# SaeedRahmani/MPC_for_AV_at_Intersection

Hardware: AMD Instinct MI355X
Metric: MPC timesteps/sec (whole node), N=20 horizon, 8-agent intersection, batch=4096 (higher is better)
Workload: dtype f64

## Files before the change

include/mpcx.h:

```cpp
#ifndef MPCX_H
#define MPCX_H
#include <stdint.h>

#ifdef __cplusplus
extern "C" {
#endif

#define MPCX_T_MAX 32
#define MPCX_MAX_PRIM 16
#define MPCX_MAX_OBS 16
#define MPCX_PRED_STEPS_MAX 64
#define MPCX_MAX_REMAINING 1024
#define MPCX_MAX_PATH_LEN 4096
#define MPCX_EGO_FRAMES_MAX 128

enum {
    MPCX_OK = 0,
    MPCX_E_INVALID = -1,
    MPCX_E_LAUNCH = -2,
    MPCX_E_NODEVICE = -3
};

enum { MPCX_QP_OPTIMAL = 0, MPCX_QP_MAXITER = 1, MPCX_QP_INFEASIBLE = 2, MPCX_QP_NUMERIC = 3 };

// ... 27 lines not shown
                            const double *u_warm ,
                            double *x_out , double *u_out ,
                            int32_t *status , int32_t *iters , double *kkt );

int32_t mpcx_mpc_prepare_batch(mpcx_ctx *ctx, int32_t B, const double *state ,
                               const double *u_warm ,
                               const double *path_xyyaw , const double *path_v ,
                               const int32_t *path_off ,
                               const int32_t *path_len , double dl, int32_t *target_ind ,
                               double *xref , uint8_t *reaches_end , double *xbar );
int32_t mpcx_mpc_prepare_batch_ov(mpcx_ctx *ctx, int32_t B, const double *state, const double *u_warm,
                                  const double *path_xyyaw, const double *path_v, const int32_t *path_off, const int32_t *path_len,
                                  double dl, int32_t *target_ind, const double *ov , int64_t ov_stride,
                                  double *xref, uint8_t *reaches_end, double *xbar);
#define MPCX_NO_STOP 999
int32_t mpcx_mpc_prepare_batch_stop(mpcx_ctx *ctx, int32_t B, const double *state, const double *u_warm,
                                    const double *path_xyyaw, const double *path_v, const int32_t *path_off, const int32_t *path_len,
                                    double dl, int32_t *target_ind, const double *ov , int64_t ov_stride,
                                    const int32_t *stop_idx , double v_ref, int32_t *len_seen ,
                                    double *xref, uint8_t *reaches_end, double *xbar);
int32_t mpcx_set_linearisation_passes(mpcx_ctx *ctx, int32_t passes);

typedef struct mpcx_search_model mpcx_search_model;
mpcx_search_model *mpcx_search_model_create(mpcx_ctx *ctx, int32_t n_prim,
                                            const int32_t *tmpl_off , const double *tmpl_xy ,
                                            const double *last_pose , const double *edge_cost ,
                                            int32_t n_obst, const int32_t *hp_off , const double *hp );
void mpcx_search_model_destroy(mpcx_search_model *m);
int32_t mpcx_expand_batch(mpcx_ctx *ctx, const mpcx_search_model *m, int32_t n_nodes, const double *nodes ,
                          const double *nodes_cs ,
                          double *nbr , double *cost , uint8_t *collide );

enum { MPCX_ASTAR_BASE = 0, MPCX_ASTAR_MODIFIED = 1, MPCX_ASTAR_MULTI_LANE = 2, MPCX_ASTAR_ROUNDABOUT = 3, MPCX_ASTAR_SINGLE_LANE = 4 };
enum { MPCX_ASTAR_FOUND = 0, MPCX_ASTAR_EXHAUSTED = 1 , MPCX_ASTAR_CAPACITY = 2, MPCX_ASTAR_MISS = 3,
       MPCX_ASTAR_PATH_CAPACITY = 4 };
typedef struct {
    double start[3];
    double goal_box[4];
    double goal_point[3];
    double allowed_dtheta;
    double wh[5];
    double wc[4];
    const double *hp_norm;
    int32_t variant;
    int32_t max_expansions;
    int32_t ov_off, ov_cnt;
} mpcx_astar_search;
typedef struct {
    int32_t heap_cap, table_cap, log_cap, push_cap, path_cap;
    double *heap, *table, *log, *push_log, *path, *cost, *miss;
    int32_t *status, *n_exp, *n_push, *path_len, *path_prim;
} mpcx_astar_buffers;
int32_t mpcx_astar_batch(mpcx_ctx *ctx, int32_t n_search, const mpcx_search_model *const *models, const mpcx_astar_search *searches,
                         int32_t n_cs, const double *cs_theta, const double *cs_val,
                         int32_t n_ov, const double *ov_key , const double *ov_val , const mpcx_astar_buffers *buffers);

int32_t mpcx_expand_multi_batch(mpcx_ctx *ctx, int32_t n_seg, const mpcx_search_model *const *models, const int32_t *seg_off,
                                const double *nodes , const double *nodes_cs ,
                                double *nbr , double *cost , uint8_t *collide );

typedef struct {
    int32_t pred_steps;
    int32_t frame_window;
    int32_t cutoff_margin;
    int32_t max_path_len;
    double dt, L, radius;
    double circle_centers[4];
    double max_accel, max_speed;
    const double *path_cum;
    double path_cum_err;
    const int32_t *path_first_within;
    const int32_t *plan_cnt;
    const double *plan_disc, *plan_box, *path_disc;
    int32_t plan_cap, plan_steps;
    double plan_dl, plan_radius;
} mpcx_interaction_params;
int32_t mpcx_interaction_batch(mpcx_ctx *ctx, const mpcx_interaction_params *ip, int32_t P,
                               const double *state ,
                               const double *path_xyyaw , const double *path_cs ,
                               const int32_t *path_off , const int32_t *path_len ,
                               const int32_t *prev_cut_len ,
                               int32_t n_obs_pool, const double *obs6 , const int32_t *obs_off ,
                               const int32_t *obs_cnt , const int32_t *obs_skip ,
                               int32_t *traj_idx , int32_t *hit_idx , double *hit_xy ,
                               int32_t *cut_len );

int32_t mpcx_moving_collision_batch(mpcx_ctx *ctx, const mpcx_interaction_params *ip, int32_t P,
                                    const double *ego_xyyaw , const double *ego_cs ,
                                    const int32_t *ego_off , const int32_t *ego_len ,
                                    const double *path_xyyaw , const double *path_cs ,
                                    const int32_t *path_off , const int32_t *path_len ,
                                    int32_t n_obs_pool, const double *obs_xyyaw , const double *obs_cs ,
                                    const int32_t *obs_off , const int32_t *obs_cnt ,
                                    int32_t *hit_idx , double *hit_xy );

int32_t mpcx_transform_batch(mpcx_ctx *ctx, int32_t n_items, int32_t max_pts, const double *nodes ,
                             const int32_t *pts_off , const int32_t *pts_cnt , const double *pts ,
                             double *out );

int32_t mpcx_cutoff_index_batch(mpcx_ctx *ctx, int32_t P, const double *pts , const int32_t *off ,
                                const int32_t *len , const double *xy , double radius, int32_t *out );

int32_t mpcx_predict_obstacles_batch(mpcx_ctx *ctx, int32_t n, int32_t steps, double dt, double L,
                                     const double *obs6 , double *out_xyyaw );

int32_t mpcx_selftest_wave_ops(mpcx_ctx *ctx, const double *in64, double *out322);
int32_t mpcx_selftest_mfma(mpcx_ctx *ctx, const double *A64, const double *B64, double *D256);

int32_t mpcx_plant_step_batch(mpcx_ctx *ctx, int32_t B, double *state , double *u ,
                              const int32_t *status , double *applied );

enum { MPCX_TRAFFIC_TINTERSECTION = 0, MPCX_TRAFFIC_ROUNDABOUT = 1, MPCX_TRAFFIC_ARTERIAL = 2, MPCX_TRAFFIC_TAPE = 3 };
typedef struct {
    int32_t kind;
    int32_t direction;
    int32_t turning;
    int32_t tape_rows, tape_off, tape_stride;
    double speed;
    double offset;
    double counter_dt;
    double model_dt;
    double L;
    double x_turn;
    double arc;
} mpcx_traffic_actor;
int32_t mpcx_traffic_step_batch(mpcx_ctx *ctx, int32_t n_actors, const mpcx_traffic_actor *actors, double *actor_state ,
                                const double *tape , int64_t tape_rows,
                                const int32_t *pool_row , int32_t n_obs_pool, double *obs6 );

typedef struct {
    int32_t P;
    int32_t exchange;
    double dl;
    double *state , *applied , *obs6 ;
    const double *path_xyyaw, *path_cs, *path_v ;
    const int32_t *path_off , *path_len , *obs_off , *obs_cnt , *obs_skip ;
    int32_t *traj_idx , *target_ind , *hit_idx , *cut_len ;
    double *hit_xy , *xref , *xbar ;
    uint8_t *reaches_end ;
    double *x_sol , *u_sol ;
    int32_t *status , *iters ;
    double *kkt ;
    int32_t n_inst, agents_local;
    double *obs_local ;
    int32_t n_actors, pool_rows ;
    const mpcx_traffic_actor *actors ;
    double *actor_state ;
    const double *tape ;
    const int32_t *actor_row , *ego_row ;
    int64_t tape_rows;
} mpcx_closed_loop;
int32_t mpcx_closed_loop_run(mpcx_ctx *ctx, const mpcx_interaction_params *ip, const mpcx_closed_loop *cl,
                             int32_t n_steps, int32_t use_graph);
int32_t mpcx_closed_loop_stats(mpcx_ctx *ctx, int64_t *out4 , int32_t reset);
int32_t mpcx_closed_loop_queue(mpcx_ctx *ctx, int32_t P, int32_t *order , int32_t *keyslot );
int32_t mpcx_interaction_prediction(mpcx_ctx *ctx, int32_t rows, int32_t steps, double *out );

typedef struct {
    int32_t capacity;
    int32_t reserved;
    double goal_dis, stop_speed;
    double *rows_f64 ;
    int32_t *rows_i32 ;
    int32_t *steps , *goal_step , *contact_step , *flags ;
    double *min_clearance ;
} mpcx_run_log;
int32_t mpcx_record_step_batch(mpcx_ctx *ctx, const mpcx_interaction_params *ip, int32_t P,
                               const double *state , const double *applied , const double *x_sol ,
                               const double *path_xyyaw , const int32_t *path_off , const int32_t *path_len ,
                               const int32_t *target_ind , const int32_t *cut_len , const int32_t *traj_idx ,
                               const int32_t *hit_idx , const int32_t *status , const int32_t *iters ,
                               int32_t n_obs_pool, const double *obs6 , const int32_t *obs_off ,
                               const int32_t *obs_cnt , const int32_t *obs_skip , const mpcx_run_log *log);
int32_t mpcx_record_step_batch_goal(mpcx_ctx *ctx, const mpcx_interaction_params *ip, int32_t P,
                                    const double *state, const double *applied, const double *x_sol,
                                    const double *path_xyyaw, const int32_t *path_off, const int32_t *path_len,
                                    const int32_t *target_ind, const int32_t *cut_len, const int32_t *traj_idx,
                                    const int32_t *hit_idx, const int32_t *status, const int32_t *iters,
                                    int32_t n_obs_pool, const double *obs6, const int32_t *obs_off,
                                    const int32_t *obs_cnt, const int32_t *obs_skip, const int32_t *goal_len ,
                                    const mpcx_run_log *log);
int32_t mpcx_closed_loop_run_logged(mpcx_ctx *ctx, const mpcx_interaction_params *ip, const mpcx_closed_loop *cl,
                                    const mpcx_run_log *log, int32_t n_steps, int32_t use_graph);
enum { MPCX_STOP_CUT = 0, MPCX_STOP_SPEED = 1 };
typedef struct {
    int32_t stop_mode;
    int32_t reserved;
    double v_ref;
    int32_t *prev_len;
} mpcx_closed_loop_opts;
int32_t mpcx_closed_loop_run_opts(mpcx_ctx *ctx, const mpcx_interaction_params *ip, const mpcx_closed_loop *cl,
                                  const mpcx_run_log *log , const mpcx_closed_loop_opts *opts ,
                                  int32_t n_steps, int32_t use_graph);

typedef struct {
    int32_t *done;
    int32_t *steps_driven;
    double goal_dis, stop_speed;
} mpcx_retire;
int32_t mpcx_closed_loop_run_retire(mpcx_ctx *ctx, const mpcx_interaction_params *ip, const mpcx_closed_loop *cl,
                                    const mpcx_run_log *log , const mpcx_closed_loop_opts *opts ,
                                    const mpcx_retire *retire , int32_t n_steps, int32_t use_graph);

typedef struct {
    int32_t *absent;
    int32_t n_rows;
    int32_t reserved;
} mpcx_scene;
int32_t mpcx_closed_loop_run_scene(mpcx_ctx *ctx, const mpcx_interaction_params *ip, const mpcx_closed_loop *cl,
                                   const mpcx_run_log *log , const mpcx_closed_loop_opts *opts ,
                                   const mpcx_retire *retire , const mpcx_scene *scene ,
                                   int32_t n_steps, int32_t use_graph);

typedef struct {
    int32_t *wait;
    int32_t *entered_step;
    int32_t *clock;
    int32_t reserved;
    double gap;
} mpcx_admit;
int32_t mpcx_closed_loop_run_admit(mpcx_ctx *ctx, const mpcx_interaction_params *ip, const mpcx_closed_loop *cl,
                                   const mpcx_run_log *log , const mpcx_closed_loop_opts *opts ,
                                   const mpcx_retire *retire , const mpcx_scene *scene ,
                                   const mpcx_admit *admit , int32_t n_steps, int32_t use_graph);
int32_t mpcx_admit_step_batch(mpcx_ctx *ctx, const mpcx_interaction_params *ip, int32_t P, const double *state ,
                              const int32_t *obs_off , const int32_t *obs_cnt , const int32_t *obs_skip ,
                              int32_t *done , int32_t n_obs_pool, int32_t *absent ,
                              int32_t n_actors, const mpcx_traffic_actor *actors , const double *actor_state ,
                              const double *tape , int64_t tape_rows, const int32_t *actor_row ,
                              const mpcx_admit *admit);

typedef struct {
    int32_t generations;
    int32_t reserved;
    const double  *start_state;
    const int32_t *start_idx;
    const int32_t *due;
    int32_t *served;
    int32_t *ep_i32;
    double  *ep_f64;
} mpcx_respawn;
int32_t mpcx_closed_loop_run_respawn(mpcx_ctx *ctx, const mpcx_interaction_params *ip, const mpcx_closed_loop *cl,
                                     const mpcx_run_log *log , const mpcx_closed_loop_opts *opts ,
                                     const mpcx_retire *retire , const mpcx_scene *scene ,
                                     const mpcx_admit *admit , const mpcx_respawn *respawn ,
                                     int32_t n_steps, int32_t use_graph);
int32_t mpcx_respawn_step_batch(mpcx_ctx *ctx, int32_t P, double *state , double *applied , double *u_sol ,
                                int32_t *traj_idx , int32_t *target_ind , int32_t *cut_len , int32_t *iters ,
                                int32_t *prev_len , const int32_t *obs_skip , int32_t n_obs_pool,
                                const mpcx_run_log *log , const mpcx_retire *retire, const mpcx_admit *admit,
                                const mpcx_respawn *respawn);

typedef struct {
    int32_t n_routes;
    int32_t reserved;
    const int32_t *route_off;
    const int32_t *route_len;
    const int32_t *route_of;
    const double  *start_state;
    const int32_t *start_idx;
    int32_t *path_off;
    int32_t *path_len;
} mpcx_routes;
int32_t mpcx_closed_loop_run_routes(mpcx_ctx *ctx, const mpcx_interaction_params *ip, const mpcx_closed_loop *cl,
                                    const mpcx_run_log *log , const mpcx_closed_loop_opts *opts ,
                                    const mpcx_retire *retire , const mpcx_scene *scene ,
                                    const mpcx_admit *admit , const mpcx_respawn *respawn ,
                                    const mpcx_routes *routes , int32_t n_steps, int32_t use_graph);
int32_t mpcx_respawn_step_batch_routes(mpcx_ctx *ctx, int32_t P, double *state , double *applied , double *u_sol ,
                                       int32_t *traj_idx , int32_t *target_ind , int32_t *cut_len , int32_t *iters ,
                                       int32_t *prev_len , const int32_t *obs_skip , int32_t n_obs_pool,
                                       const mpcx_run_log *log , const mpcx_retire *retire, const mpcx_admit *admit,
                                       const mpcx_respawn *respawn, const mpcx_routes *routes , int32_t max_path_len);
int32_t mpcx_episode_summary(mpcx_ctx *ctx, int32_t P, int32_t A, int32_t G, int32_t R, const int32_t *served ,
                             const int32_t *ep_i32 , const double *ep_f64 , int64_t *out_i64 ,
                             double *out_f64 );

enum { MPCX_PRECEDENCE_FIXED = 1, MPCX_PRECEDENCE_ENTRY = 2 };
typedef struct {
    int32_t *prec;
    double *stand;
    int32_t n_rows;
    int32_t mode;
} mpcx_precedence;
int32_t mpcx_closed_loop_run_precedence(mpcx_ctx *ctx, const mpcx_interaction_params *ip, const mpcx_closed_loop *cl,
                                        const mpcx_run_log *log , const mpcx_closed_loop_opts *opts ,
                                        const mpcx_retire *retire , const mpcx_scene *scene ,
                                        const mpcx_admit *admit , const mpcx_respawn *respawn ,
                                        const mpcx_routes *routes , const mpcx_precedence *precedence ,
                                        int32_t n_steps, int32_t use_graph);
int32_t mpcx_admit_step_batch_precedence(mpcx_ctx *ctx, const mpcx_interaction_params *ip, int32_t P, const double *state ,
                                         const int32_t *obs_off , const int32_t *obs_cnt , const int32_t *obs_skip ,
                                         int32_t *done , int32_t n_obs_pool, int32_t *absent ,
                                         int32_t n_actors, const mpcx_traffic_actor *actors , const double *actor_state ,
                                         const double *tape , int64_t tape_rows, const int32_t *actor_row ,
                                         const mpcx_admit *admit, const mpcx_precedence *precedence );

#define MPCX_SIGNAL_GROUPS_MAX 16
typedef struct {
    const int32_t *path_stop;
    const int32_t *path_group;
    const int32_t *plan_cycle;
    const int32_t *plan_amber;
    const int32_t *plan_green;
    const int32_t *plan_of;
    int32_t *tick;
// ... 70 lines not shown
```

mpc_for_av_at_intersection_amd/_lib.py:

```python
import ctypes as C
import os

_HERE = os.path.dirname(os.path.abspath(__file__))
LIB_PATH = os.environ.get('MPCX_LIB') or os.path.join(_HERE, 'libmpcx.so')
_lib = None

c_dp = C.c_void_p


MODEL_BICYCLE4, MODEL_JERK5 = 0, 1


class MpcParamsC(C.Structure):
    _fields_ = [('T', C.c_int32), ('max_iter', C.c_int32), ('dt', C.c_double), ('L', C.c_double),
                ('w_perp', C.c_double), ('w_para', C.c_double), ('R', C.c_double * 2), ('Rd', C.c_double * 2),
                ('Q_v_yaw', C.c_double * 2), ('Qf', C.c_double * 4), ('R_end', C.c_double * 2),
                ('max_speed', C.c_double), ('min_speed', C.c_double), ('max_accel', C.c_double),
                ('max_decel', C.c_double), ('max_steer', C.c_double), ('max_dsteer', C.c_double), ('tol', C.c_double),
                ('model', C.c_int32), ('reserved', C.c_int32), ('jerk_weight', C.c_double)]


class InteractionParamsC(C.Structure):
    _fields_ = [('pred_steps', C.c_int32), ('frame_window', C.c_int32),
                ('cutoff_margin', C.c_int32), ('max_path_len', C.c_int32), ('dt', C.c_double), ('L', C.c_double), ('radius', C.c_double),
                ('circle_centers', C.c_double * 4), ('max_accel', C.c_double), ('max_speed', C.c_double),
                ('path_cum', C.c_void_p), ('path_cum_err', C.c_double), ('path_first_within', C.c_void_p),
                ('plan_cnt', C.c_void_p), ('plan_disc', C.c_void_p), ('plan_box', C.c_void_p), ('path_disc', C.c_void_p),
                ('plan_cap', C.c_int32), ('plan_steps', C.c_int32), ('plan_dl', C.c_double), ('plan_radius', C.c_double)]


class ClosedLoopC(C.Structure):
    _PTRS = ['state', 'applied', 'obs6', 'path_xyyaw', 'path_cs', 'path_v', 'path_off', 'path_len', 'obs_off', 'obs_cnt',
             'obs_skip', 'traj_idx', 'target_ind', 'hit_idx', 'cut_len', 'hit_xy', 'xref', 'xbar', 'reaches_end',
             'x_sol', 'u_sol', 'status', 'iters', 'kkt']
    _fields_ = ([('P', C.c_int32), ('exchange', C.c_int32), ('dl', C.c_double)] + [(n, C.c_void_p) for n in _PTRS] +
                [('n_inst', C.c_int32), ('agents_local', C.c_int32), ('obs_local', C.c_void_p)] +
                [('n_actors', C.c_int32), ('pool_rows', C.c_int32), ('actors', C.c_void_p), ('actor_state', C.c_void_p), ('tape', C.c_void_p),
                 ('actor_row', C.c_void_p), ('ego_row', C.c_void_p), ('tape_rows', C.c_int64)])


class RunLogC(C.Structure):
    _fields_ = ([('capacity', C.c_int32), ('reserved', C.c_int32), ('goal_dis', C.c_double), ('stop_speed', C.c_double)] +
                [(n, C.c_void_p) for n in ('rows_f64', 'rows_i32', 'steps', 'goal_step', 'contact_step', 'flags', 'min_clearance')])


class ClosedLoopOptsC(C.Structure):
    _fields_ = [('stop_mode', C.c_int32), ('reserved', C.c_int32), ('v_ref', C.c_double), ('prev_len', C.c_void_p)]


class RetireC(C.Structure):
    _fields_ = [('done', C.c_void_p), ('steps_driven', C.c_void_p), ('goal_dis', C.c_double), ('stop_speed', C.c_double)]


class SceneC(C.Structure):
    _fields_ = [('absent', C.c_void_p), ('n_rows', C.c_int32), ('reserved', C.c_int32)]


class AdmitC(C.Structure):
    _fields_ = [('wait', C.c_void_p), ('entered_step', C.c_void_p), ('clock', C.c_void_p), ('reserved', C.c_int32), ('gap', C.c_double)]


class RespawnC(C.Structure):
    _fields_ = [('generations', C.c_int32), ('reserved', C.c_int32), ('start_state', C.c_void_p), ('start_idx', C.c_void_p), ('due', C.c_void_p),
                ('served', C.c_void_p), ('ep_i32', C.c_void_p), ('ep_f64', C.c_void_p)]


class RoutesC(C.Structure):
    _fields_ = [('n_routes', C.c_int32), ('reserved', C.c_int32), ('route_off', C.c_void_p), ('route_len', C.c_void_p), ('route_of', C.c_void_p),
                ('start_state', C.c_void_p), ('start_idx', C.c_void_p), ('path_off', C.c_void_p), ('path_len', C.c_void_p)]


class PrecedenceC(C.Structure):
    _fields_ = [('prec', C.c_void_p), ('stand', C.c_void_p), ('n_rows', C.c_int32), ('mode', C.c_int32)]


PRECEDENCE_FIXED, PRECEDENCE_ENTRY = 1, 2
PRECEDENCE_WINDOW = 64
PRECEDENCE_MAX_STEP = (2 ** 31 - 1 - (PRECEDENCE_WINDOW - 1)) // PRECEDENCE_WINDOW


class SignalsC(C.Structure):
    _fields_ = [('path_stop', C.c_void_p), ('path_group', C.c_void_p), ('plan_cycle', C.c_void_p), ('plan_amber', C.c_void_p),
                ('plan_green', C.c_void_p), ('plan_of', C.c_void_p), ('tick', C.c_void_p), ('held', C.c_void_p), ('brake', C.c_double),
                ('n_points', C.c_int32), ('n_plans', C.c_int32), ('n_groups', C.c_int32), ('reserved', C.c_int32)]


class ActuationC(C.Structure):
    _fields_ = [('phase_groups', C.c_void_p), ('phase_time', C.c_void_p), ('ctrl_time', C.c_void_p), ('ctrl_of', C.c_void_p),
                ('jstate', C.c_void_p), ('lights', C.c_void_p), ('calls', C.c_void_p), ('n_per', C.c_int32), ('n_junctions', C.c_int32),
                ('n_phases', C.c_int32), ('n_ctrl', C.c_int32), ('reserved', C.c_int32)]


SIGNAL_GROUPS_MAX = 16
ACTUATION_PHASES_MAX = 8
STAGE_GREEN, STAGE_AMBER, STAGE_ALL_RED = 0, 1, 2
LIGHT_GREEN, LIGHT_AMBER, LIGHT_RED = 0, 1, 2
HELD_FREE, HELD_RED, HELD_AMBER = 0, 1, 2


EPISODE_I32 = ('entered', 'arrived', 'steps_driven', 'row_end', 'contact_step', 'flags', 'due')
EPISODE_F64 = ('min_clearance',)
EPISODE_ROUTE_WORD = 7
SUMMARY_I64 = ('count', 'contacts', 'delay_sum', 'steps_driven_sum')


STOP_CUT, STOP_SPEED = 0, 1
STOP_MODES = {'cut': STOP_CUT, 'speed': STOP_SPEED}
NO_STOP = 999


RUN_LOG_F64 = ('x', 'y', 'v', 'yaw', 'accel', 'steer', 'xref_deviation', 'clearance')
RUN_LOG_I32 = ('traj_idx', 'target_ind', 'cut_len', 'hit_idx', 'status', 'iters')
RUN_LOG_ROW_BYTES = 96
RUN_LOG_AGENT_BYTES = 24


class TrafficActorC(C.Structure):
    _fields_ = ([(n, C.c_int32) for n in ('kind', 'direction', 'turning', 'tape_rows', 'tape_off', 'tape_stride')] +
                [(n, C.c_double) for n in ('speed', 'offset', 'counter_dt', 'model_dt', 'L', 'x_turn', 'arc')])


class AstarSearchC(C.Structure):
    _fields_ = [('start', C.c_double * 3), ('goal_box', C.c_double * 4), ('goal_point', C.c_double * 3), ('allowed_dtheta', C.c_double),
                ('wh', C.c_double * 5), ('wc', C.c_double * 4), ('hp_norm', C.c_void_p),
                ('variant', C.c_int32), ('max_expansions', C.c_int32), ('ov_off', C.c_int32), ('ov_cnt', C.c_int32)]


class AstarBuffersC(C.Structure):
    _fields_ = ([(n, C.c_int32) for n in ('heap_cap', 'table_cap', 'log_cap', 'push_cap', 'path_cap')] +
                [(n, C.c_void_p) for n in ('heap', 'table', 'log', 'push_log', 'path', 'cost', 'miss', 'status', 'n_exp', 'n_push', 'path_len', 'path_prim')])


import numpy as _np
ASTAR_SEARCH_DTYPE = _np.dtype([('start', '<f8', 3), ('goal_box', '<f8', 4), ('goal_point', '<f8', 3), ('allowed_dtheta', '<f8'),
                                ('wh', '<f8', 5), ('wc', '<f8', 4), ('hp_norm', '<u8'), ('variant', '<i4'), ('max_expansions', '<i4'),
                                ('ov_off', '<i4'), ('ov_cnt', '<i4')])
assert ASTAR_SEARCH_DTYPE.itemsize == C.sizeof(AstarSearchC)
TRAFFIC_ACTOR_DTYPE = _np.dtype([(n, '<i4') for n in ('kind', 'direction', 'turning', 'tape_rows', 'tape_off', 'tape_stride')] +
                                [(n, '<f8') for n in ('speed', 'offset', 'counter_dt', 'model_dt', 'L', 'x_turn', 'arc')])
assert TRAFFIC_ACTOR_DTYPE.itemsize == C.sizeof(TrafficActorC)
TRAFFIC_TINTERSECTION, TRAFFIC_ROUNDABOUT, TRAFFIC_ARTERIAL, TRAFFIC_TAPE = 0, 1, 2, 3
MAX_OBS = 16
ASTAR_BASE, ASTAR_MODIFIED, ASTAR_MULTI_LANE, ASTAR_ROUNDABOUT, ASTAR_SINGLE_LANE = 0, 1, 2, 3, 4
ASTAR_VARIANTS = {'base': ASTAR_BASE, 'modified': ASTAR_MODIFIED, 'multi_lane': ASTAR_MULTI_LANE, 'roundabout': ASTAR_ROUNDABOUT,
                  'single_lane': ASTAR_SINGLE_LANE}
ASTAR_FOUND, ASTAR_EXHAUSTED, ASTAR_CAPACITY, ASTAR_MISS, ASTAR_PATH_CAPACITY = 0, 1, 2, 3, 4
COMM_ID_BYTES = 128
SHARD_INSTANCES, SHARD_AGENTS = 1, 2


EXPORTS = ['mpcx_create', 'mpcx_destroy', 'mpcx_last_error', 'mpcx_version', 'mpcx_set_mpc_params',
           'mpcx_qp_solve_batch', 'mpcx_mpc_prepare_batch', 'mpcx_search_model_create', 'mpcx_search_model_destroy',
           'mpcx_expand_batch', 'mpcx_interaction_batch', 'mpcx_moving_collision_batch', 'mpcx_plant_step_batch',
           'mpcx_transform_batch', 'mpcx_cutoff_index_batch', 'mpcx_predict_obstacles_batch', 'mpcx_selftest_wave_ops', 'mpcx_selftest_mfma',
           'mpcx_closed_loop_run', 'mpcx_profile_qp', 'mpcx_profile_qp_read', 'mpcx_set_instance_tuning', 'mpcx_set_qp_solver', 'mpcx_qp_set_order_hint', 'mpcx_expand_multi_batch',
           'mpcx_comm_unique_id', 'mpcx_comm_init', 'mpcx_comm_destroy', 'mpcx_allgather_states', 'mpcx_closed_loop_stats',
           'mpcx_mpc_prepare_batch_ov', 'mpcx_set_linearisation_passes', 'mpcx_astar_batch', 'mpcx_traffic_step_batch',
           'mpcx_record_step_batch', 'mpcx_closed_loop_run_logged', 'mpcx_mpc_prepare_batch_stop', 'mpcx_record_step_batch_goal',
           'mpcx_closed_loop_run_opts', 'mpcx_closed_loop_run_retire', 'mpcx_closed_loop_run_scene', 'mpcx_closed_loop_run_admit',
           'mpcx_admit_step_batch', 'mpcx_closed_loop_run_respawn', 'mpcx_respawn_step_batch', 'mpcx_closed_loop_run_routes',
           'mpcx_respawn_step_batch_routes', 'mpcx_episode_summary', 'mpcx_closed_loop_run_precedence', 'mpcx_admit_step_batch_precedence',
           'mpcx_closed_loop_run_signals', 'mpcx_signal_step_batch', 'mpcx_closed_loop_queue', 'mpcx_interaction_prediction',
           'mpcx_closed_loop_run_actuated', 'mpcx_actuated_step_batch']


def load():
    global _lib
    if _lib is not None:
        return _lib
    if not os.path.exists(LIB_PATH):
        raise RuntimeError('libmpcx.so not built (%s): run `python -c "import __graft_entry__ as g; g.build()"` '
                           'or `make -C mpc_for_av_at_intersection_amd/csrc`; there is no CPU fallback' % LIB_PATH)
    import torch
    lib = C.CDLL(LIB_PATH)
    vp, i32 = C.c_void_p, C.c_int32
    lib.mpcx_create.restype = vp; lib.mpcx_create.argtypes = [i32, vp]
    lib.mpcx_destroy.restype = None; lib.mpcx_destroy.argtypes = [vp]
    lib.mpcx_last_error.restype = C.c_char_p; lib.mpcx_last_error.argtypes = [vp]
    lib.mpcx_version.restype = C.c_char_p; lib.mpcx_version.argtypes = []
    lib.mpcx_set_mpc_params.restype = i32; lib.mpcx_set_mpc_params.argtypes = [vp, C.POINTER(MpcParamsC)]
    lib.mpcx_qp_solve_batch.restype = i32; lib.mpcx_qp_solve_batch.argtypes = [vp, i32] + [vp] * 10
    lib.mpcx_mpc_prepare_batch.restype = i32
    lib.mpcx_mpc_prepare_batch.argtypes = [vp, i32, vp, vp, vp, vp, vp, vp, C.c_double, vp, vp, vp, vp]
    lib.mpcx_mpc_prepare_batch_ov.restype = i32
    lib.mpcx_mpc_prepare_batch_ov.argtypes = [vp, i32, vp, vp, vp, vp, vp, vp, C.c_double, vp, vp, C.c_int64, vp, vp, vp]
    lib.mpcx_set_linearisation_passes.restype = i32; lib.mpcx_set_linearisation_passes.argtypes = [vp, i32]
    lib.mpcx_astar_batch.restype = i32
    lib.mpcx_astar_batch.argtypes = [vp, i32, vp, vp, i32, vp, vp, i32, vp, vp, vp]
    lib.mpcx_search_model_create.restype = vp
    lib.mpcx_search_model_create.argtypes = [vp, i32, vp, vp, vp, vp, i32, vp, vp]
    lib.mpcx_search_model_destroy.restype = None; lib.mpcx_search_model_destroy.argtypes = [vp]
    lib.mpcx_expand_batch.restype = i32; lib.mpcx_expand_batch.argtypes = [vp, vp, i32, vp, vp, vp, vp, vp]
    lib.mpcx_interaction_batch.restype = i32
    lib.mpcx_interaction_batch.argtypes = [vp, C.POINTER(InteractionParamsC), i32] + [vp] * 6 + [i32] + [vp] * 8
    lib.mpcx_moving_collision_batch.restype = i32
    lib.mpcx_moving_collision_batch.argtypes = [vp, C.POINTER(InteractionParamsC), i32] + [vp] * 8 + [i32] + [vp] * 6
    lib.mpcx_plant_step_batch.restype = i32; lib.mpcx_plant_step_batch.argtypes = [vp, i32, vp, vp, vp, vp]
    lib.mpcx_transform_batch.restype = i32; lib.mpcx_transform_batch.argtypes = [vp, i32, i32, vp, vp, vp, vp, vp]
    lib.mpcx_cutoff_index_batch.restype = i32
    lib.mpcx_cutoff_index_batch.argtypes = [vp, i32, vp, vp, vp, vp, C.c_double, vp]
    lib.mpcx_predict_obstacles_batch.restype = i32
    lib.mpcx_predict_obstacles_batch.argtypes = [vp, i32, i32, C.c_double, C.c_double, vp, vp]
    lib.mpcx_selftest_wave_ops.restype = i32; lib.mpcx_selftest_wave_ops.argtypes = [vp, vp, vp]
    lib.mpcx_selftest_mfma.restype = i32; lib.mpcx_selftest_mfma.argtypes = [vp, vp, vp, vp]
    lib.mpcx_closed_loop_run.restype = i32
    lib.mpcx_closed_loop_run.argtypes = [vp, C.POINTER(InteractionParamsC), C.POINTER(ClosedLoopC), i32, i32]
    lib.mpcx_profile_qp.restype = i32; lib.mpcx_profile_qp.argtypes = [vp, i32]
    lib.mpcx_profile_qp_read.restype = i32
    lib.mpcx_profile_qp_read.argtypes = [vp, C.POINTER(C.c_double), C.POINTER(C.c_int32)]
    lib.mpcx_set_instance_tuning.restype = i32; lib.mpcx_set_instance_tuning.argtypes = [vp, vp, i32]
    lib.mpcx_set_qp_solver.restype = i32; lib.mpcx_set_qp_solver.argtypes = [vp, i32]
    lib.mpcx_qp_set_order_hint.restype = i32; lib.mpcx_qp_set_order_hint.argtypes = [vp, vp, vp, vp]
    lib.mpcx_expand_multi_batch.restype = i32; lib.mpcx_expand_multi_batch.argtypes = [vp, i32, vp, vp, vp, vp, vp, vp, vp]
    lib.mpcx_comm_unique_id.restype = i32; lib.mpcx_comm_unique_id.argtypes = [vp]
    lib.mpcx_comm_init.restype = i32; lib.mpcx_comm_init.argtypes = [vp, i32, i32, vp]
    lib.mpcx_comm_destroy.restype = i32; lib.mpcx_comm_destroy.argtypes = [vp]
    lib.mpcx_allgather_states.restype = i32; lib.mpcx_allgather_states.argtypes = [vp, i32, i32, i32, vp, vp]
    lib.mpcx_closed_loop_stats.restype = i32; lib.mpcx_closed_loop_stats.argtypes = [vp, C.POINTER(C.c_int64), i32]
    lib.mpcx_closed_loop_queue.restype = i32; lib.mpcx_closed_loop_queue.argtypes = [vp, i32, vp, vp]
    lib.mpcx_interaction_prediction.restype = i32; lib.mpcx_interaction_prediction.argtypes = [vp, i32, i32, vp]
    lib.mpcx_traffic_step_batch.restype = i32; lib.mpcx_traffic_step_batch.argtypes = [vp, i32, vp, vp, vp, C.c_int64, vp, i32, vp]
    lib.mpcx_record_step_batch.restype = i32
    lib.mpcx_record_step_batch.argtypes = [vp, C.POINTER(InteractionParamsC), i32] + [vp] * 12 + [i32] + [vp] * 4 + [C.POINTER(RunLogC)]
    lib.mpcx_closed_loop_run_logged.restype = i32
    lib.mpcx_closed_loop_run_logged.argtypes = [vp, C.POINTER(InteractionParamsC), C.POINTER(ClosedLoopC), C.POINTER(RunLogC), i32, i32]
    lib.mpcx_mpc_prepare_batch_stop.restype = i32
    lib.mpcx_mpc_prepare_batch_stop.argtypes = [vp, i32, vp, vp, vp, vp, vp, vp, C.c_double, vp, vp, C.c_int64, vp, C.c_double, vp, vp, vp, vp]
    lib.mpcx_record_step_batch_goal.restype = i32
    lib.mpcx_record_step_batch_goal.argtypes = [vp, C.POINTER(InteractionParamsC), i32] + [vp] * 12 + [i32] + [vp] * 5 + [C.POINTER(RunLogC)]
    lib.mpcx_closed_loop_run_opts.restype = i32
    lib.mpcx_closed_loop_run_opts.argtypes = [vp, C.POINTER(InteractionParamsC), C.POINTER(ClosedLoopC), C.POINTER(RunLogC),
                                              C.POINTER(ClosedLoopOptsC), i32, i32]
    lib.mpcx_closed_loop_run_retire.restype = i32
    lib.mpcx_closed_loop_run_retire.argtypes = [vp, C.POINTER(InteractionParamsC), C.POINTER(ClosedLoopC), C.POINTER(RunLogC),
                                                C.POINTER(ClosedLoopOptsC), C.POINTER(RetireC), i32, i32]
    lib.mpcx_closed_loop_run_scene.restype = i32
    lib.mpcx_closed_loop_run_scene.argtypes = [vp, C.POINTER(InteractionParamsC), C.POINTER(ClosedLoopC), C.POINTER(RunLogC),
                                               C.POINTER(ClosedLoopOptsC), C.POINTER(RetireC), C.POINTER(SceneC), i32, i32]
    lib.mpcx_closed_loop_run_admit.restype = i32
    lib.mpcx_closed_loop_run_admit.argtypes = [vp, C.POINTER(InteractionParamsC), C.POINTER(ClosedLoopC), C.POINTER(RunLogC),
                                               C.POINTER(ClosedLoopOptsC), C.POINTER(RetireC), C.POINTER(SceneC), C.POINTER(AdmitC), i32, i32]
    lib.mpcx_admit_step_batch.restype = i32
    lib.mpcx_admit_step_batch.argtypes = [vp, C.POINTER(InteractionParamsC), i32, vp, vp, vp, vp, vp, i32, vp, i32, vp, vp, vp, C.c_int64, vp,
                                          C.POINTER(AdmitC)]
    lib.mpcx_closed_loop_run_respawn.restype = i32
    lib.mpcx_closed_loop_run_respawn.argtypes = [vp, C.POINTER(InteractionParamsC), C.POINTER(ClosedLoopC), C.POINTER(RunLogC),
                                                 C.POINTER(ClosedLoopOptsC), C.POINTER(RetireC), C.POINTER(SceneC), C.POINTER(AdmitC),
                                                 C.POINTER(RespawnC), i32, i32]
    lib.mpcx_respawn_step_batch.restype = i32
    lib.mpcx_respawn_step_batch.argtypes = [vp, i32] + [vp] * 9 + [i32, C.POINTER(RunLogC), C.POINTER(RetireC), C.POINTER(AdmitC),
                                                                   C.POINTER(RespawnC)]
    lib.mpcx_closed_loop_run_routes.restype = i32
    lib.mpcx_closed_loop_run_routes.argtypes = [vp, C.POINTER(InteractionParamsC), C.POINTER(ClosedLoopC), C.POINTER(RunLogC),
                                                C.POINTER(ClosedLoopOptsC), C.POINTER(RetireC), C.POINTER(SceneC), C.POINTER(AdmitC),
                                                C.POINTER(RespawnC), C.POINTER(RoutesC), i32, i32]
    lib.mpcx_respawn_step_batch_routes.restype = i32
    lib.mpcx_respawn_step_batch_routes.argtypes = [vp, i32] + [vp] * 9 + [i32, C.POINTER(RunLogC), C.POINTER(RetireC), C.POINTER(AdmitC),
                                                                          C.POINTER(RespawnC), C.POINTER(RoutesC), i32]
    lib.mpcx_episode_summary.restype = i32
    lib.mpcx_episode_summary.argtypes = [vp, i32, i32, i32, i32, vp, vp, vp, vp, vp]
    lib.mpcx_closed_loop_run_precedence.restype = i32
    lib.mpcx_closed_loop_run_precedence.argtypes = [vp, C.POINTER(InteractionParamsC), C.POINTER(ClosedLoopC), C.POINTER(RunLogC),
                                                    C.POINTER(ClosedLoopOptsC), C.POINTER(RetireC), C.POINTER(SceneC), C.POINTER(AdmitC),
                                                    C.POINTER(RespawnC), C.POINTER(RoutesC), C.POINTER(PrecedenceC), i32, i32]
    lib.mpcx_admit_step_batch_precedence.restype = i32
    lib.mpcx_admit_step_batch_precedence.argtypes = [vp, C.POINTER(InteractionParamsC), i32, vp, vp, vp, vp, vp, i32, vp, i32, vp, vp, vp,
                                                     C.c_int64, vp, C.POINTER(AdmitC), C.POINTER(PrecedenceC)]
    lib.mpcx_closed_loop_run_signals.restype = i32
    lib.mpcx_closed_loop_run_signals.argtypes = [vp, C.POINTER(InteractionParamsC), C.POINTER(ClosedLoopC), C.POINTER(RunLogC),
                                                 C.POINTER(ClosedLoopOptsC), C.POINTER(RetireC), C.POINTER(SceneC), C.POINTER(AdmitC),
                                                 C.POINTER(RespawnC), C.POINTER(RoutesC), C.POINTER(PrecedenceC), C.POINTER(SignalsC), i32, i32]
    lib.mpcx_signal_step_batch.restype = i32
    lib.mpcx_signal_step_batch.argtypes = [vp, i32, C.c_double, vp, vp, vp, vp, vp, vp, C.POINTER(SignalsC)]
    lib.mpcx_closed_loop_run_actuated.restype = i32
    lib.mpcx_closed_loop_run_actuated.argtypes = [vp, C.POINTER(InteractionParamsC), C.POINTER(ClosedLoopC), C.POINTER(RunLogC),
                                                  C.POINTER(ClosedLoopOptsC), C.POINTER(RetireC), C.POINTER(SceneC), C.POINTER(AdmitC),
                                                  C.POINTER(RespawnC), C.POINTER(RoutesC), C.POINTER(PrecedenceC), C.POINTER(SignalsC),
                                                  C.POINTER(ActuationC), i32, i32]
    lib.mpcx_actuated_step_batch.restype = i32
    lib.mpcx_actuated_step_batch.argtypes = [vp, i32, C.c_double, vp, vp, vp, vp, vp, vp, C.POINTER(SignalsC), C.POINTER(ActuationC)]
    _lib = lib
    return lib
```

mpc_for_av_at_intersection_amd/csrc/mpcx_api.hip:

```cpp
#include "mpcx_common.h"
#include <cstdarg>
#include <cstdio>
#include <new>

int32_t mpcx_fail(mpcx_ctx *ctx, int32_t code, const char *fmt, ...) {
    if (ctx) {
        va_list ap;
        va_start(ap, fmt);
        vsnprintf(ctx->err, sizeof ctx->err, fmt, ap);
        va_end(ap);
    }
    return code;
}

int32_t mpcx_check_launch(mpcx_ctx *ctx, const char *what) {
    hipError_t e = hipGetLastError();
    if (e != hipSuccess) return mpcx_fail(ctx, MPCX_E_LAUNCH, "%s: %s", what, hipGetErrorString(e));
    return MPCX_OK;
}

int32_t mpcx_grow(mpcx_ctx *ctx, void **p, size_t *cap_bytes, size_t need_bytes, const char *what) {
    if (need_bytes <= *cap_bytes) return MPCX_OK;
    if (*p) (void)hipFree(*p);
    *p = nullptr; *cap_bytes = 0;
    if (hipMalloc(p, need_bytes) != hipSuccess) return mpcx_fail(ctx, MPCX_E_LAUNCH, "cannot allocate %zu bytes for %s", need_bytes, what);
    *cap_bytes = need_bytes;
    return MPCX_OK;
}

extern "C" {

const char *mpcx_version(void) { return "mpcx 0.1 (gfx950)"; }

mpcx_ctx *mpcx_create(int32_t device, void *hip_stream) {
    int n = 0;
    if (hipGetDeviceCount(&n) != hipSuccess || n <= 0 || device < 0 || device >= n) return nullptr;
    if (hipSetDevice(device) != hipSuccess) return nullptr;
    mpcx_ctx *c = new (std::nothrow) mpcx_ctx();
    if (!c) return nullptr;
    c->device = device;
    c->stream = (hipStream_t)hip_stream;
    hipDeviceProp_t prop;
    c->n_cu = (hipGetDeviceProperties(&prop, device) == hipSuccess && prop.multiProcessorCount > 0) ? prop.multiProcessorCount : 256;
    if (hipStreamCreateWithFlags(&c->side, hipStreamNonBlocking) != hipSuccess ||
        hipEventCreateWithFlags(&c->ev_fork, hipEventDisableTiming) != hipSuccess ||
        hipEventCreateWithFlags(&c->ev_join, hipEventDisableTiming) != hipSuccess) { mpcx_destroy(c); return nullptr; }
    return c;
}

void mpcx_destroy(mpcx_ctx *ctx) {
    if (!ctx) return;
    if (ctx->loop_exec) { (void)hipStreamSynchronize(ctx->stream); (void)hipGraphExecDestroy(ctx->loop_exec); }
    for (hipEvent_t e : ctx->prof_ev) (void)hipEventDestroy(e);
    for (hipEvent_t e : ctx->prof_free) (void)hipEventDestroy(e);
    if (ctx->order) (void)hipFree(ctx->order);
    if (ctx->multi) (void)hipFree(ctx->multi);
    if (ctx->cs) (void)hipFree(ctx->cs);
    if (ctx->side) { (void)hipStreamSynchronize(ctx->side); (void)hipStreamDestroy(ctx->side); }
    if (ctx->ev_fork) (void)hipEventDestroy(ctx->ev_fork);
    if (ctx->ev_join) (void)hipEventDestroy(ctx->ev_join);
    if (ctx->prev_cut) (void)hipFree(ctx->prev_cut);
    if (ctx->bins) (void)hipFree(ctx->bins);
    if (ctx->pred) (void)hipFree(ctx->pred);
    if (ctx->ticket) (void)hipFree(ctx->ticket);
    (void)mpcx_comm_destroy(ctx);
    if (ctx->stats) (void)hipFree(ctx->stats);
    if (ctx->xchg) (void)hipFree(ctx->xchg);
    if (ctx->admit_tab) (void)hipFree(ctx->admit_tab);
    delete ctx;
}

const char *mpcx_last_error(mpcx_ctx *ctx) { return ctx ? ctx->err : "null context"; }

int32_t mpcx_set_mpc_params(mpcx_ctx *ctx, const mpcx_mpc_params *p) {
    if (!ctx || !p) return MPCX_E_INVALID;
    if (p->T < 1 || p->T > MPCX_T_MAX) return mpcx_fail(ctx, MPCX_E_INVALID, "horizon T=%d outside 1..%d", p->T, MPCX_T_MAX);
    if (!(p->dt > 0) || !(p->L > 0) || p->max_iter < 1 || !(p->tol > 0))
        return mpcx_fail(ctx, MPCX_E_INVALID, "dt, L, tol must be positive and max_iter >= 1");
    if (p->model != MPCX_MODEL_BICYCLE4 && p->model != MPCX_MODEL_JERK5)
        return mpcx_fail(ctx, MPCX_E_INVALID, "model %d: MPCX_MODEL_BICYCLE4 (lib/mpc.py) or MPCX_MODEL_JERK5 (lib/mpc_jerk.py)", p->model);
    if (p->model == MPCX_MODEL_JERK5 && !(p->jerk_weight >= 0.0))
        return mpcx_fail(ctx, MPCX_E_INVALID, "jerk_weight must be >= 0");
    ctx->mpc = *p;
    ctx->have_mpc = true;
    return MPCX_OK;
}

int32_t mpcx_set_instance_tuning(mpcx_ctx *ctx, const mpcx_qp_tuning *rows, int32_t n_rows) {
    if (!ctx) return MPCX_E_INVALID;
    if ((rows == nullptr) != (n_rows == 0) || n_rows < 0)
        return mpcx_fail(ctx, MPCX_E_INVALID, "set_instance_tuning: rows and n_rows must both be given or both be empty");
    ctx->tune = rows;
    ctx->tune_rows = n_rows;
    return MPCX_OK;
}

int32_t mpcx_qp_set_order_hint(mpcx_ctx *ctx, const int32_t *prev_iters, const int32_t *ref_now, const int32_t *ref_prev) {
    if (!ctx) return MPCX_E_INVALID;
    if ((ref_now == nullptr) != (ref_prev == nullptr))
        return mpcx_fail(ctx, MPCX_E_INVALID, "qp_set_order_hint: ref_now and ref_prev come as a pair");
    ctx->order_hint = prev_iters;
    ctx->order_now = ref_now;
    ctx->order_prev = ref_prev;
    return MPCX_OK;
}

int32_t mpcx_set_qp_solver(mpcx_ctx *ctx, int32_t which) {
    if (!ctx) return MPCX_E_INVALID;
    if (which < 0 || which > 2) return mpcx_fail(ctx, MPCX_E_INVALID, "set_qp_solver: 0 (automatic), 1 (condensed) or 2 (stage-structured)");
    ctx->qp_solver = which;
    return MPCX_OK;
}

int32_t mpcx_set_linearisation_passes(mpcx_ctx *ctx, int32_t passes) {
    if (!ctx) return MPCX_E_INVALID;
    if (passes < 1 || passes > 16) return mpcx_fail(ctx, MPCX_E_INVALID, "set_linearisation_passes: 1..16 (lib/mpc.py MAX_ITER)");
    ctx->lin_passes = passes;
    return MPCX_OK;
}

int32_t mpcx_profile_qp(mpcx_ctx *ctx, int32_t enable) {
    if (!ctx) return MPCX_E_INVALID;
    ctx->prof_qp = enable != 0;
    return MPCX_OK;
}

int32_t mpcx_profile_qp_read(mpcx_ctx *ctx, double *total_ms, int32_t *launches) {
    if (!ctx || !total_ms || !launches) return MPCX_E_INVALID;
    double sum = 0.0;
    const size_t n = ctx->prof_ev.size() / 2;
    for (size_t i = 0; i < n; i++) {
        float ms = 0.f;
        if (hipEventSynchronize(ctx->prof_ev[2 * i + 1]) != hipSuccess ||
            hipEventElapsedTime(&ms, ctx->prof_ev[2 * i], ctx->prof_ev[2 * i + 1]) != hipSuccess)
            return mpcx_fail(ctx, MPCX_E_LAUNCH, "profile_qp_read: event %zu could not be read", i);
        sum += ms;
    }
    ctx->prof_free.insert(ctx->prof_free.end(), ctx->prof_ev.begin(), ctx->prof_ev.end());
    ctx->prof_ev.clear();
    *total_ms = sum;
    *launches = (int32_t)n;
    return MPCX_OK;
}

}
```

mpc_for_av_at_intersection_amd/csrc/mpcx_common.h:

```cpp
#pragma once
#include <hip/hip_runtime.h>
#include <stdint.h>
#include "mpcx.h"
#include "mpcx_qp_consts.h"
#include <vector>

struct mpcx_ctx {
    int device = 0;
    hipStream_t stream = nullptr;
    mpcx_mpc_params mpc = {};
    bool have_mpc = false;
    int32_t *ticket = nullptr;
    int n_cu = 0;
    double *pred = nullptr;
    size_t pred_cap = 0;
    hipGraphExec_t loop_exec = nullptr;
    unsigned char loop_key[1272] = {};
    const mpcx_qp_tuning *tune = nullptr;
    int32_t tune_rows = 0;
    const int32_t *order_hint = nullptr;
    const int32_t *order_now = nullptr, *order_prev = nullptr;
    int32_t *prev_cut = nullptr;
    size_t prev_cut_cap = 0;
    int32_t *order = nullptr;
    size_t order_cap = 0;
    int32_t *bins = nullptr;
    size_t bins_cap = 0;
    bool bins_clean = false;
    hipStream_t side = nullptr;
    hipEvent_t ev_fork = nullptr, ev_join = nullptr;
    double *cs = nullptr;
    size_t cs_cap = 0;
    void *multi = nullptr;
    size_t multi_cap = 0;
    int qp_solver = 0;
    int lin_passes = 1;
    bool prof_qp = false;
    std::vector<hipEvent_t> prof_ev;
    std::vector<hipEvent_t> prof_free;
    unsigned long long *stats = nullptr;
    size_t stats_slots = 0;
    void *comm = nullptr;
    int comm_world = 1, comm_rank = 0;
    double *xchg = nullptr;
    size_t xchg_cap = 0;
    double *admit_tab = nullptr;
    size_t admit_tab_cap = 0;
    char err[256] = {};
};

struct mpcx_interaction_extras {
    const double *pack_state = nullptr, *pack_applied = nullptr;
    const int32_t *ego_row = nullptr, *actor_row = nullptr;
    int32_t n_ego = 0, n_actors = 0;
    int32_t *prev_save = nullptr;
    const int32_t *key_prev = nullptr;
    int32_t *near = nullptr;
    const int32_t *bin_hint = nullptr;
    const int32_t *done = nullptr;
    const int32_t *absent = nullptr;
    const int32_t *prec = nullptr;
    double *stand = nullptr;
};
struct mpcx_window_extras {
    bool scatter = false;
    const int32_t *near = nullptr, *tidx = nullptr;
    bool rollout_forked = false;
    const int32_t *stop_idx = nullptr;
    double v_ref = 0.0;
    int32_t *len_seen = nullptr;
    const int32_t *done = nullptr;
    int32_t *queue_len = nullptr;
};
struct mpcx_qp_order {
    bool ready = false;
    const int32_t *hint = nullptr, *now = nullptr, *prev = nullptr;
    const int32_t *queue_len = nullptr;
};
struct mpcx_plant_extras {
    const int32_t *stats_iters = nullptr;
    bool reset_bins = false;
    const int32_t *done = nullptr;
};
int32_t mpcx_interaction_enqueue(mpcx_ctx *ctx, const mpcx_interaction_params *ip, int32_t P, const double *state, const double *path_xyyaw,
                               const double *path_cs, const int32_t *path_off, const int32_t *path_len, const int32_t *prev_cut_len,
                               int32_t n_obs_pool, const double *obs6, const int32_t *obs_off, const int32_t *obs_cnt, const int32_t *obs_skip,
                               int32_t *traj_idx, int32_t *hit_idx, double *hit_xy, int32_t *cut_len, const mpcx_interaction_extras &x);
int32_t mpcx_window_enqueue(mpcx_ctx *ctx, int32_t B, const double *state, const double *u_warm, const double *path_xyyaw, const double *path_v,
                          const int32_t *path_off, const int32_t *path_len, double dl, int32_t *target_ind, const double *ov, int64_t ov_stride,
                          double *xref, uint8_t *reaches_end, double *xbar, const mpcx_window_extras &x);
int32_t mpcx_qp_enqueue(mpcx_ctx *ctx, int32_t B, const double *x0, const double *xref, const double *xbar, const uint8_t *reaches_end,
                      const double *u_warm, double *x_out, double *u_out, int32_t *status, int32_t *iters, double *kkt, const mpcx_qp_order &ord);
int32_t mpcx_plant_enqueue(mpcx_ctx *ctx, int32_t B, double *state, double *u, const int32_t *status, double *applied, const mpcx_plant_extras &x);

int32_t mpcx_fail(mpcx_ctx *ctx, int32_t code, const char *fmt, ...);
int32_t mpcx_check_launch(mpcx_ctx *ctx, const char *what);
int32_t mpcx_grow(mpcx_ctx *ctx, void **p, size_t *cap_bytes, size_t need_bytes, const char *what);
int32_t mpcx_ensure_pred(mpcx_ctx *ctx, size_t need_doubles);
int32_t mpcx_rollout_fork(mpcx_ctx *ctx, int32_t B, const double *state, const double *u_warm, double *xbar, const int32_t *done = nullptr);
int32_t mpcx_traffic_validate(mpcx_ctx *ctx, int32_t n_actors, const mpcx_traffic_actor *actors, const double *tape, int64_t tape_rows,
                              const int32_t *pool_row, int32_t n_obs_pool);
int32_t mpcx_traffic_enqueue(mpcx_ctx *ctx, int32_t n_actors, const mpcx_traffic_actor *actors, double *actor_state, const double *tape,
                             int64_t tape_rows, const int32_t *pool_row, int32_t n_obs_pool, double *obs6);
bool mpcx_record_absent(const mpcx_run_log *log);
int32_t mpcx_record_validate(mpcx_ctx *ctx, const mpcx_run_log *log, const int32_t *obs_skip);
int32_t mpcx_record_enqueue(mpcx_ctx *ctx, const mpcx_interaction_params *ip, int32_t P, const double *state, const double *applied,
                            const double *x_sol, const double *path_xyyaw, const int32_t *path_off, const int32_t *path_len,
                            const int32_t *target_ind, const int32_t *cut_len, const int32_t *traj_idx, const int32_t *hit_idx,
                            const int32_t *status, const int32_t *iters, int32_t n_obs_pool, const double *obs6, const int32_t *obs_off,
                            const int32_t *obs_cnt, const int32_t *obs_skip, const mpcx_run_log *log,
                            const int32_t *goal_len = nullptr,
                            const int32_t *done = nullptr,
                            const int32_t *absent = nullptr);
bool mpcx_retire_absent(const mpcx_retire *r);
int32_t mpcx_retire_validate(mpcx_ctx *ctx, const mpcx_retire *r, int32_t P);
int32_t mpcx_retire_enqueue(mpcx_ctx *ctx, int32_t P, const double *state, double *applied, const double *path_xyyaw, const int32_t *path_off,
                            const int32_t *path_len, const int32_t *target_ind, const int32_t *goal_len, const mpcx_retire *r,
                            const mpcx_scene *scene = nullptr, const int32_t *own_row = nullptr);
bool mpcx_scene_absent(const mpcx_scene *s);
int32_t mpcx_scene_validate(mpcx_ctx *ctx, const mpcx_scene *s, const mpcx_retire *retire, int32_t exchange, size_t pool_rows, const int32_t *obs_skip);
bool mpcx_admit_absent(const mpcx_admit *a);
int32_t mpcx_admit_validate(mpcx_ctx *ctx, const mpcx_admit *a, const mpcx_retire *retire, const mpcx_scene *scene, int32_t exchange);
int32_t mpcx_admit_prepare(mpcx_ctx *ctx, size_t n_rows);
int32_t mpcx_admit_enqueue(mpcx_ctx *ctx, const mpcx_interaction_params *ip, int32_t P, const double *state, const int32_t *obs_off,
                           const int32_t *obs_cnt, const int32_t *obs_skip, int32_t *done, int32_t n_obs_pool, int32_t *absent,
                           int32_t n_actors, const mpcx_traffic_actor *actors, const double *actor_state, const double *tape,
                           int64_t tape_rows, const int32_t *actor_row, const mpcx_admit *admit);
bool mpcx_respawn_absent(const mpcx_respawn *s);
int32_t mpcx_respawn_validate(mpcx_ctx *ctx, const mpcx_respawn *s, const mpcx_admit *admit);
int32_t mpcx_respawn_enqueue(mpcx_ctx *ctx, int32_t P, double *state, double *applied, double *u_sol, int32_t *traj_idx, int32_t *target_ind,
                             int32_t *cut_len, int32_t *iters, int32_t *prev_len , const int32_t *obs_skip, int32_t n_obs_pool,
                             const mpcx_run_log *log , const mpcx_retire *retire, const mpcx_admit *admit,
                             const mpcx_respawn *respawn);
bool mpcx_routes_absent(const mpcx_routes *s);
int32_t mpcx_routes_validate(mpcx_ctx *ctx, const mpcx_routes *s, const mpcx_respawn *respawn, const int32_t *path_off, const int32_t *path_len,
                             int32_t max_len );
int32_t mpcx_route_enqueue(mpcx_ctx *ctx, int32_t P, double *state, double *applied, double *u_sol, int32_t *traj_idx, int32_t *target_ind,
                           int32_t *cut_len, int32_t *iters, int32_t *prev_len , const int32_t *obs_skip, int32_t n_obs_pool,
                           const mpcx_run_log *log , const mpcx_retire *retire, const mpcx_admit *admit,
                           const mpcx_respawn *respawn, const mpcx_routes *routes);
bool mpcx_precedence_absent(const mpcx_precedence *s);
int32_t mpcx_precedence_validate(mpcx_ctx *ctx, const mpcx_precedence *s, const mpcx_scene *scene, const mpcx_admit *admit);
int32_t mpcx_precedence_enqueue(mpcx_ctx *ctx, int32_t P, const int32_t *obs_off, const int32_t *obs_skip, const mpcx_admit *admit,
                                const mpcx_precedence *precedence);
bool mpcx_signals_absent(const mpcx_signals *s);
int32_t mpcx_signals_validate(mpcx_ctx *ctx, const mpcx_signals *s, int32_t exchange);
int32_t mpcx_signal_enqueue(mpcx_ctx *ctx, int32_t P, double dl, const double *state, const int32_t *path_off, const int32_t *path_len,
                            const int32_t *traj_idx, int32_t *cut_len, const int32_t *done , const mpcx_signals *signals);
bool mpcx_actuation_absent(const mpcx_actuation *s);
int32_t mpcx_actuation_validate(mpcx_ctx *ctx, const mpcx_actuation *s, const mpcx_signals *sg, int32_t P, int32_t exchange);
int32_t mpcx_actuated_enqueue(mpcx_ctx *ctx, int32_t P, double dl, const double *state, const int32_t *path_off, const int32_t *path_len,
                              const int32_t *traj_idx, int32_t *cut_len, const int32_t *done , const mpcx_signals *signals,
                              const mpcx_actuation *actuation);
int32_t mpcx_ensure_ticket(mpcx_ctx *ctx);
#define MPCX_JUMP_BONUS 11
#define MPCX_ORDER_BINS 64
#define MPCX_TICKET_WORDS 8
#define MPCX_TICKET_QUEUE_LEN 6
#define MPCX_ORDER_COPIES 16
namespace mpcx {
__device__ __forceinline__ int order_key_of(int hint, bool moved) {
    int k = hint < 0 ? 0 : hint;
    if (moved) k += MPCX_JUMP_BONUS;
    return k < MPCX_ORDER_BINS ? k : MPCX_ORDER_BINS - 1;
}
}
int32_t mpcx_ensure_order(mpcx_ctx *ctx, size_t B);
int32_t mpcx_qp_build_order(mpcx_ctx *ctx, int32_t B, const int32_t *hint, const int32_t *now, const int32_t *prev, hipStream_t st);

namespace mpcx {

constexpr int WAVE = 64;

struct QpArgs {
    mpcx_mpc_params p;
    int B;
    int32_t *ticket;
    int has_warm;
    const double *x0, *xref, *xbar, *u_warm;
    const uint8_t *re;
    double *x_out, *u_out, *kkt;
    int32_t *status, *iters;
    const mpcx_qp_tuning *tune;
    int has_tune;
    const int32_t *order;
    int has_order;
    int defer_fail;
    int32_t *fail_list, *fail_count;
    const int32_t *queue_len;
    int has_queue_len;
};

void launch_qp_stage(const QpArgs &a, hipStream_t st, int n_cu);
int qp_stage_grid(int B, int n_cu);

__device__ __forceinline__ double rdlane(double v, int l) {
    int lo = __double2loint(v), hi = __double2hiint(v);
    lo = __builtin_amdgcn_readlane(lo, l);
    hi = __builtin_amdgcn_readlane(hi, l);
    return __hiloint2double(hi, lo);
}
__device__ __forceinline__ double frcp(double d) {
    double r = __builtin_amdgcn_rcp(d);
    r = fma(fma(-d, r, 1.0), r, r);
    r = fma(fma(-d, r, 1.0), r, r);
    return r;
}

template <int CTRL, int ROW_MASK = 0xF>
__device__ __forceinline__ double dpp_mov(double old, double src) {
    int lo = __builtin_amdgcn_update_dpp(__double2loint(old), __double2loint(src), CTRL, ROW_MASK, 0xF, false);
    int hi = __builtin_amdgcn_update_dpp(__double2hiint(old), __double2hiint(src), CTRL, ROW_MASK, 0xF, false);
    return __hiloint2double(hi, lo);
}
__device__ __forceinline__ double lane_next(double v, double fill = 0.0) { return dpp_mov<0x130>(fill, v); }
__device__ __forceinline__ double lane_prev(double v, double fill = 0.0) { return dpp_mov<0x138>(fill, v); }

__device__ __forceinline__ double scan_up32(double v) {
    v += dpp_mov<0x111>(0.0, v);
    v += dpp_mov<0x112>(0.0, v);
    v += dpp_mov<0x114>(0.0, v);
    v += dpp_mov<0x118>(0.0, v);
    v += dpp_mov<0x142, 0xA>(0.0, v);
    return v;
}
__device__ __forceinline__ double scan_down32(double v, int lane) {
    v += dpp_mov<0x101>(0.0, v);
    v += dpp_mov<0x102>(0.0, v);
    v += dpp_mov<0x104>(0.0, v);
    v += dpp_mov<0x108>(0.0, v);
    const double r1 = rdlane(v, 16);
    return v + ((lane < 16) ? r1 : 0.0);
}
__device__ __forceinline__ double wave_sum_dpp(double v) {
    v += dpp_mov<0x111>(0.0, v);
    v += dpp_mov<0x112>(0.0, v);
    v += dpp_mov<0x114>(0.0, v);
    v += dpp_mov<0x118>(0.0, v);
    return (rdlane(v, 15) + rdlane(v, 31)) + (rdlane(v, 47) + rdlane(v, 63));
}
__device__ __forceinline__ double wave_max_dpp(double v) {
    v = fmax(v, dpp_mov<0x111>(v, v));
    v = fmax(v, dpp_mov<0x112>(v, v));
    v = fmax(v, dpp_mov<0x114>(v, v));
    v = fmax(v, dpp_mov<0x118>(v, v));
    return fmax(fmax(rdlane(v, 15), rdlane(v, 31)), fmax(rdlane(v, 47), rdlane(v, 63)));
// ... 121 lines not shown
```

mpc_for_av_at_intersection_amd/csrc/mpcx_interaction.hip:

```cpp
#include "mpcx_common.h"

namespace mpcx {

#ifdef MPCX_INTER_FORCE_EXACT
constexpr bool FORCE_EXACT = true;
#else
constexpr bool FORCE_EXACT = false;
#endif

__device__ __forceinline__ void pose_discs(const mpcx_interaction_params &ip, double px, double py, double c, double s, double *out) {
#pragma unroll
    for (int d = 0; d < 2; d++) disc_centre(px, py, c, s, ip.circle_centers[2 * d], ip.circle_centers[2 * d + 1], out[2 * d], out[2 * d + 1]);
}

struct PredArgs {
    mpcx_interaction_params ip;
    int n, n_pool;
    const double *obs6;
    double *pred;
    const double *pack_state, *pack_applied;
    double *pack_out;
    const int32_t *ego_row, *actor_row;
    int n_ego;
    const int32_t *absent;
    double *stand;
};

template <bool MAPPED, bool SCENE = false, bool STAND = false>
__global__ __launch_bounds__(256) void predict_kernel(PredArgs a) {
    int o = blockIdx.x * blockDim.x + threadIdx.x;
    if (o >= a.n) return;
    double x, y, v, yaw, acc, steer;
    bool pack = a.pack_state != nullptr;
    int src = o;
    if constexpr (MAPPED) {
        pack = o < a.n_ego;
        o = pack ? a.ego_row[o] : a.actor_row[o - a.n_ego];
        if (o < 0 || o >= a.n_pool) return;
    }
    if (pack) {
        const double *st = a.pack_state + 4 * (size_t)src;
        x = st[0]; y = st[1]; v = st[2]; yaw = st[3]; acc = a.pack_applied[2 * src + 1]; steer = a.pack_applied[2 * src];
        double *row = a.pack_out + 6 * (size_t)o;
        row[0] = x; row[1] = y; row[2] = v; row[3] = yaw; row[4] = acc; row[5] = steer;
    } else {
        const double *s6 = a.obs6 + 6 * (size_t)o;
        x = s6[0]; y = s6[1]; v = s6[2]; yaw = s6[3]; acc = s6[4]; steer = s6[5];
    }
    if constexpr (SCENE) { if (a.absent[o] != 0) return; }
    const double tn = tan(steer);
    const double dt = a.ip.dt;
    double s, c;
    sincos(yaw, &s, &c);
    if constexpr (STAND) pose_discs(a.ip, x, y, c, s, a.stand + 4 * (size_t)o);
    double *out = a.pred + (size_t)o * a.ip.pred_steps * 4;
    for (int k = 0; k < a.ip.pred_steps; k++) {
        x = __dadd_rn(x, __dmul_rn(__dmul_rn(v, c), dt));
        y = __dadd_rn(y, __dmul_rn(__dmul_rn(v, s), dt));
        v = __dadd_rn(v, __dmul_rn(acc, dt));
        yaw = __dadd_rn(yaw, __dmul_rn(__dmul_rn(__ddiv_rn(v, a.ip.L), tn), dt));
        sincos(yaw, &s, &c);
        pose_discs(a.ip, x, y, c, s, out + 4 * k);
    }
}

struct InterArgs {
    mpcx_interaction_params ip;
    int P;
    const double *state, *path, *path_cs;
    const int32_t *path_off, *path_len, *prev_cut;
    const double *pred;
    const int32_t *obs_off, *obs_cnt, *obs_skip;
    int32_t *traj_idx, *hit_idx;
    double *hit_xy;
    int32_t *cut_len;
    int max_rem, fcap;
    int32_t *prev_save;
    const int32_t *bin_hint;
    int32_t *bin_cnt, *keyslot;
    const int32_t *key_prev;
    int32_t *near;
    const int32_t *done;
    const int32_t *absent;
    int n_rows;
    const int32_t *prec;
    const double *stand;
};

__device__ __forceinline__ double dist2d(double ax, double ay, double bx, double by) {
    const double dx = __dadd_rn(ax, -bx), dy = __dadd_rn(ay, -by);
    return __dsqrt_rn(__dadd_rn(__dmul_rn(dx, dx), __dmul_rn(dy, dy)));
}
struct Within {
    double md, md2lo, md2hi;
    __device__ __forceinline__ explicit Within(double md_) : md(md_), md2lo(md_ * md_ * (1.0 - 1e-12)), md2hi(md_ * md_ * (1.0 + 1e-12)) {}
    __device__ __forceinline__ bool operator()(double ax, double ay, double bx, double by) const {
        const double dx = __dadd_rn(ax, -bx), dy = __dadd_rn(ay, -by);
        const double d2 = __dadd_rn(__dmul_rn(dx, dx), __dmul_rn(dy, dy));
        if (d2 > md2hi) return false;
        if (d2 < md2lo) return true;
        return __dsqrt_rn(d2) <= md;
    }
};

constexpr int NSEG = 8;
constexpr int SPARE_ROWS = 32;
__device__ __forceinline__ double grp8_min(double v) {
    v = fmin(v, dpp_mov<0xB1>(v, v)); v = fmin(v, dpp_mov<0x4E>(v, v)); v = fmin(v, dpp_mov<0x141>(v, v));
    return v;
}
__device__ __forceinline__ double grp8_max(double v) {
    v = fmax(v, dpp_mov<0xB1>(v, v)); v = fmax(v, dpp_mov<0x4E>(v, v)); v = fmax(v, dpp_mov<0x141>(v, v));
    return v;
}
__device__ __forceinline__ void divmod_small(int j, int d, float inv_d, int &quo, int &rem) {
    int q = (int)(((float)j + 0.5f) * inv_d);
    int r = j - q * d;
    if (r < 0) { q -= 1; r += d; }
    if (r >= d) { q += 1; r -= d; }
    quo = q; rem = r;
}

__device__ __forceinline__ void run_boxes(const double (*s_ego)[4], int na, int F, int SL, double slack, double (*s_box)[4], int lane) {
    const int sg = lane >> 3, j = lane & 7;
    const int fend = (sg + 1) * SL < F ? (sg + 1) * SL : F;
    double x0 = INFINITY, x1 = -INFINITY, y0 = INFINITY, y1 = -INFINITY;
    for (int f = sg * SL + j; f < fend; f += 8) {
        const int fe = f < na ? f : na - 1;
#pragma unroll
        for (int d = 0; d < 2; d++) {
            const double ex = s_ego[fe][2 * d], ey = s_ego[fe][2 * d + 1];
            x0 = fmin(x0, ex); x1 = fmax(x1, ex); y0 = fmin(y0, ey); y1 = fmax(y1, ey);
        }
    }
    x0 = grp8_min(x0); x1 = grp8_max(x1); y0 = grp8_min(y0); y1 = grp8_max(y1);
    if (j == 0) { s_box[sg][0] = x0 - slack; s_box[sg][1] = x1 + slack; s_box[sg][2] = y0 - slack; s_box[sg][3] = y1 + slack; }
}

struct RowList {
    unsigned long long lo, hi;
    static constexpr int PER = 10, BITS = 6;
    static_assert(MPCX_MAX_OBS <= PER + 64 / BITS, "two words do not hold the list");
    static __device__ __forceinline__ RowList of(unsigned long long m) {
        RowList l = {0, 0};
        for (int r = 0; m; r++, m &= m - 1) {
            const unsigned long long k = (unsigned long long)(__ffsll((long long)m) - 1);
            if (r < PER) l.lo |= k << (BITS * r); else l.hi |= k << (BITS * (r - PER));
        }
        return l;
    }
    __device__ __forceinline__ int operator[](int o) const {
        const bool first = o < PER;
        return (int)(((first ? lo : hi) >> (BITS * (first ? o : o - PER))) & 63ull);
    }
};
template <bool SCENE = false, bool PREC = false>
__device__ __forceinline__ bool first_row(const mpcx_interaction_params &ip, const Within &within, const double (*s_ego)[4], int na, int F, int SL,
                                          const double (*s_box)[4], const double *pred, int ooff, int nobs, int oskip, int lane,
                                          double &hox, double &hoy, const RowList rows = {0, 0}, const double *stand = nullptr,
                                          unsigned yields = 0u) {
    const int steps = ip.pred_steps, w = ip.frame_window;
    const float inv_steps = 1.0f / (float)steps;
    const long long NOKEY = 0x7fffffffffffffffLL;
    long long lbest = NOKEY;
    double lpx = 0.0, lpy = 0.0;
    int sg_limit = NSEG;
    const int ncand_all = nobs * steps * 2;
    for (int cb = 0; cb < ncand_all; cb += 8 * WAVE) {
        double ox[8], oy[8];
#pragma unroll
        for (int u = 0; u < 8; u++) {
            const int cidx = cb + u * WAVE + lane;
            const int cc = cidx < ncand_all ? cidx : ncand_all - 1;
            const int co = cc & 1;
            int g, o;
            divmod_small(cc >> 1, steps, inv_steps, o, g);
            int pool;
            if constexpr (SCENE) pool = ooff + rows[o];
            else {
                pool = ooff + o;
                if (oskip >= 0 && pool >= oskip) pool += 1;
            }
            const double *qq = pred + ((size_t)pool * steps + g) * 4 + 2 * co;
            if constexpr (PREC) {
                const double *qs = stand + (size_t)pool * 4 + 2 * co;
                qq = ((yields >> o) & 1u) ? qs : qq;
            }
            ox[u] = qq[0]; oy[u] = qq[1];
        }
#pragma unroll
        for (int u = 0; u < 8; u++)
            if (cb + u * WAVE + lane >= ncand_all) { ox[u] = INFINITY; oy[u] = INFINITY; }
        for (int sg = 0; sg < sg_limit; sg++) {
            const double b0 = s_box[sg][0], b1 = s_box[sg][1], b2 = s_box[sg][2], b3 = s_box[sg][3];
            unsigned mask = 0;
#pragma unroll
            for (int u = 0; u < 8; u++)
                mask |= (unsigned)((ox[u] >= b0) & (ox[u] <= b1) & (oy[u] >= b2) & (oy[u] <= b3)) << u;
            if (!__ballot(mask != 0u)) continue;
            const int f0 = sg * SL;
            int f1 = (sg + 1) * SL < F ? (sg + 1) * SL : F;
            bool found = false;
            while (__ballot(mask != 0u)) {
                const bool on = mask != 0u;
                const int u = on ? __ffs((int)mask) - 1 : 0;
                mask &= mask - 1;
                double px = ox[0], py = oy[0];
#pragma unroll
                for (int q = 1; q < 8; q++) { px = (u == q) ? ox[q] : px; py = (u == q) ? oy[q] : py; }
                const int cidx = cb + u * WAVE + lane;
                const int co = cidx & 1;
                int g, o;
                divmod_small(cidx >> 1, steps, inv_steps, o, g);
                for (int f = f0; f < f1; f++) {
                    const int ff = f < steps ? f : steps - 1;
                    const int fe = f < na ? f : na - 1;
// ... 432 lines not shown
}
__device__ __forceinline__ unsigned yields_by_rank(unsigned long long present, unsigned long long yielding) {
    unsigned out = 0u;
    for (unsigned long long m = yielding; m; m &= m - 1) {
        const int k = __ffsll((long long)m) - 1;
        out |= 1u << __popcll(present & ((1ull << k) - 1ull));
    }
    return out;
}

template <bool RETIRE, bool SCENE = false, bool PREC = false>
__global__ __launch_bounds__(64, 5) void interaction_kernel(InterArgs a) {
    static_assert(!PREC || (RETIRE && SCENE), "precedence lives on a scene");
    if constexpr (RETIRE) { if (a.done[blockIdx.x] != 0) return; }
    extern __shared__ double s_dyn[];
    const int MAXREM = a.max_rem, MAXF = a.fcap;
    double *s_cum = s_dyn;
    unsigned short *s_keep = reinterpret_cast<unsigned short *>(s_dyn + MAXREM);
    double (*s_ego)[4] = reinterpret_cast<double (*)[4]>(s_cum);
    double (*s_box)[4] = reinterpret_cast<double (*)[4]>(s_cum + (size_t)MAXF * 4);

    const int p = blockIdx.x, lane = threadIdx.x;
    const mpcx_interaction_params &ip = a.ip;
    const size_t poff = (size_t)a.path_off[p];
    const double *path = a.path + 3 * poff;
    const int len = a.path_len[p];
    const double x = a.state[4 * p], y = a.state[4 * p + 1], v = a.state[4 * p + 2];
    const int t_old = a.traj_idx[p];
    const int pcut = a.prev_cut ? a.prev_cut[p] : 0;
    const int kprev = a.key_prev ? a.key_prev[p] : pcut;
    if (a.prev_save && lane == 0) a.prev_save[p] = kprev;
    int nobs;
    RowList rows = {0, 0};
    unsigned yields = 0u;
    if constexpr (SCENE) {
        const int cnt = a.obs_cnt[p];
        const unsigned long long present = present_rows(a, p, lane, cnt, a.obs_off[p], a.obs_skip ? a.obs_skip[p] : -1);
        nobs = cnt > WAVE ? MPCX_MAX_OBS + 1 : __popcll(present);
        if (nobs <= MPCX_MAX_OBS) rows = RowList::of(present);
        if constexpr (PREC) {
            if (nobs <= MPCX_MAX_OBS) yields = yields_by_rank(present, yielding_rows(a, lane, cnt, a.obs_off[p], a.obs_skip ? a.obs_skip[p] : -1, present));
        }
    } else
        nobs = a.obs_cnt[p] - ((a.obs_skip && a.obs_skip[p] >= 0) ? 1 : 0);
    const double *cumtab = ip.path_cum ? ip.path_cum + poff : nullptr;

    const int tidx = locate(a, p, lane, path, len, t_old, x, y, pcut, nobs, cumtab != nullptr, s_cum);
    if (tidx < 0) { leave(a, p, lane, kprev, len, tidx); return; }
    if (lane == 0) a.traj_idx[p] = tidx;
    if (nobs <= 0) { leave(a, p, lane, kprev, len, -1); return; }
    __syncthreads();

    const double dl_const = __dmul_rn(ip.dt, ip.max_speed);
    const Ego e{ip, lane, MAXF, s_cum, s_keep, cumtab,
                path + 3 * (size_t)tidx,
                tidx, tidx - t_old, len - tidx, v, v < ip.max_speed, dl_const, frcp(dl_const),
                cumtab ? cumtab[tidx] : 0.0, cumtab ? ip.path_cum_err + 1e-13 : 1.01e-10};
    const double *rcs = a.path_cs + 2 * (poff + tidx);
    const size_t prow = poff + tidx;
    bool from_plan;
    const int na = ego_frames(e, prow, s_ego, s_box, from_plan);
    if (na > MAXF) { leave(a, p, lane, kprev, len, -2); return; }
    __syncthreads();
    if (!from_plan) ego_discs(e, rcs, na, s_ego);
    __syncthreads();
    const int ooff = a.obs_off[p], oskip = a.obs_skip ? a.obs_skip[p] : -1;
    double hx, hy;
    const double *pdisc = ip.plan_cnt ? ip.path_disc + 4 * prow : nullptr;
    const int first = first_conflict<SCENE, PREC>(ip, s_ego, na, a.pred, ooff, nobs, oskip, e.rem, rcs, e.n, s_box, lane, hx, hy, from_plan, pdisc, rows,
                                                  a.stand, yields);
    if (first < 0) { leave(a, p, lane, kprev, len, -1); return; }
    finish(a, p, lane, kprev, first, hx, hy, cut_index(ip, path, poff, len, tidx, tidx + first, hx, hy, lane));
}

void launch_predict_stand(bool mapped, int lanes, hipStream_t st, const PredArgs &pa);
void launch_interaction_prec(int P, size_t lds, hipStream_t st, const InterArgs &ia);

#ifndef MPCX_INTERACTION_TEMPLATES_ONLY
struct PoseDiscArgs {
    mpcx_interaction_params ip;
    int n;
    const double *pose, *cs;
    double *out;
};
__global__ __launch_bounds__(256) void pose_disc_kernel(PoseDiscArgs a) {
    const int i = blockIdx.x * blockDim.x + threadIdx.x;
    if (i >= a.n) return;
    const double px = a.pose[3 * i], py = a.pose[3 * i + 1], c = a.cs[2 * i], s = a.cs[2 * i + 1];
    pose_discs(a.ip, px, py, c, s, a.out + 4 * i);
}

struct MovArgs {
    mpcx_interaction_params ip;
    int P;
    const double *ego, *ego_cs;
    const int32_t *ego_off, *ego_len;
    const double *path, *path_cs;
    const int32_t *path_off, *path_len;
    const double *pred;
    const int32_t *obs_off, *obs_cnt;
    int32_t *hit_idx;
    double *hit_xy;
};

__global__ __launch_bounds__(64) void moving_collision_kernel(MovArgs a) {
    __shared__ double s_ego[MPCX_EGO_FRAMES_MAX][4];
    __shared__ double s_box[NSEG][4];
    const int p = blockIdx.x, lane = threadIdx.x;
    const mpcx_interaction_params &ip = a.ip;
    const int na = a.ego_len[p], n = a.path_len[p], nobs = a.obs_cnt[p];
    if (nobs <= 0) { if (lane == 0) { a.hit_idx[p] = -1; a.hit_xy[2 * p] = 0; a.hit_xy[2 * p + 1] = 0; } return; }
    if (na > MPCX_EGO_FRAMES_MAX || na < 1 || n < 1 || nobs > MPCX_MAX_OBS) { if (lane == 0) { a.hit_idx[p] = -2; a.hit_xy[2 * p] = 0; a.hit_xy[2 * p + 1] = 0; } return; }
    const double *ego = a.ego + 3 * (size_t)a.ego_off[p], *ecs = a.ego_cs + 2 * (size_t)a.ego_off[p];
    for (int f = lane; f < na; f += WAVE) {
        const double px = ego[3 * f], py = ego[3 * f + 1], c = ecs[2 * f], s = ecs[2 * f + 1];
        pose_discs(ip, px, py, c, s, s_ego[f]);
    }
    __syncthreads();
    double hx, hy;
    const int first = first_conflict(ip, s_ego, na, a.pred, a.obs_off[p], nobs, -1,
                                     a.path + 3 * (size_t)a.path_off[p], a.path_cs + 2 * (size_t)a.path_off[p], n, s_box, lane, hx, hy);
    if (lane == 0) { a.hit_idx[p] = first; a.hit_xy[2 * p] = first < 0 ? 0.0 : hx; a.hit_xy[2 * p + 1] = first < 0 ? 0.0 : hy; }
}
#endif

}

#ifndef MPCX_INTERACTION_TEMPLATES_ONLY

extern "C" int32_t mpcx_interaction_batch(mpcx_ctx *ctx, const mpcx_interaction_params *ip, int32_t P,
                                          const double *state, const double *path_xyyaw, const double *path_cs,
                                          const int32_t *path_off, const int32_t *path_len, const int32_t *prev_cut_len,
                                          int32_t n_obs_pool, const double *obs6, const int32_t *obs_off,
                                          const int32_t *obs_cnt, const int32_t *obs_skip,
                                          int32_t *traj_idx, int32_t *hit_idx, double *hit_xy, int32_t *cut_len) {
    return mpcx_interaction_enqueue(ctx, ip, P, state, path_xyyaw, path_cs, path_off, path_len, prev_cut_len, n_obs_pool, obs6, obs_off,
                                    obs_cnt, obs_skip, traj_idx, hit_idx, hit_xy, cut_len, {});
}

int32_t mpcx_interaction_enqueue(mpcx_ctx *ctx, const mpcx_interaction_params *ip, int32_t P, const double *state, const double *path_xyyaw,
                                 const double *path_cs, const int32_t *path_off, const int32_t *path_len, const int32_t *prev_cut_len,
                                 int32_t n_obs_pool, const double *obs6, const int32_t *obs_off, const int32_t *obs_cnt, const int32_t *obs_skip,
                                 int32_t *traj_idx, int32_t *hit_idx, double *hit_xy, int32_t *cut_len, const mpcx_interaction_extras &x) {
    if (!ctx) return MPCX_E_INVALID;
    if (P == 0) return MPCX_OK;
    if (!ip || P < 0 || n_obs_pool < 0 || !state || !path_xyyaw || !path_cs || !path_off || !path_len || !obs_off ||
        !obs_cnt || !traj_idx || !hit_idx || !hit_xy || !cut_len || (n_obs_pool > 0 && !obs6))
        return mpcx_fail(ctx, MPCX_E_INVALID, "interaction_batch: null pointer or negative size");
    if (ip->pred_steps < 1 || ip->pred_steps > MPCX_PRED_STEPS_MAX || ip->frame_window < 0 || !(ip->dt > 0) || !(ip->L > 0))
        return mpcx_fail(ctx, MPCX_E_INVALID, "interaction_batch: pred_steps outside 1..%d or bad dt/L/frame_window", MPCX_PRED_STEPS_MAX);
    if (x.absent && (!x.done || n_obs_pool < 1)) return mpcx_fail(ctx, MPCX_E_INVALID, "interaction_batch: a scene without retirement or without a pool");
    if ((x.prec || x.stand) && (!x.absent || !x.prec || !x.stand)) return mpcx_fail(ctx, MPCX_E_INVALID, "interaction_batch: precedence without a scene, or without one of prec and stand");
    { int32_t rc = mpcx_ensure_pred(ctx, (size_t)(n_obs_pool > 0 ? n_obs_pool : 1) * ip->pred_steps * 4); if (rc != MPCX_OK) return rc; }
    if (n_obs_pool > 0 && x.pack_state && x.ego_row) {
        const int lanes = x.n_ego + x.n_actors;
        mpcx::PredArgs pa{*ip, lanes, n_obs_pool, obs6, ctx->pred, x.pack_state, x.pack_applied, const_cast<double *>(obs6),
                          x.ego_row, x.actor_row, x.n_ego, x.absent, x.stand};
        if (x.prec) mpcx::launch_predict_stand(true, lanes, ctx->stream, pa);
        else if (x.absent) hipLaunchKernelGGL((mpcx::predict_kernel<true, true>), dim3((lanes + 63) / 64), dim3(64), 0, ctx->stream, pa);
        else hipLaunchKernelGGL(mpcx::predict_kernel<true>, dim3((lanes + 63) / 64), dim3(64), 0, ctx->stream, pa);
    } else if (n_obs_pool > 0) {
        mpcx::PredArgs pa{*ip, n_obs_pool, n_obs_pool, obs6, ctx->pred, x.pack_state, x.pack_applied, x.pack_state ? const_cast<double *>(obs6) : nullptr,
                          nullptr, nullptr, 0, x.absent, x.stand};
        if (x.prec) mpcx::launch_predict_stand(false, n_obs_pool, ctx->stream, pa);
        else if (x.absent) hipLaunchKernelGGL((mpcx::predict_kernel<false, true>), dim3((n_obs_pool + 63) / 64), dim3(64), 0, ctx->stream, pa);
        else hipLaunchKernelGGL(mpcx::predict_kernel<false>, dim3((n_obs_pool + 63) / 64), dim3(64), 0, ctx->stream, pa);
    }
    int max_rem = ip->max_path_len > 0 ? ip->max_path_len : MPCX_MAX_REMAINING;
    if (max_rem < 512) max_rem = 512;
    max_rem = (max_rem + 63) / 64 * 64;
    if (max_rem > MPCX_MAX_PATH_LEN)
        return mpcx_fail(ctx, MPCX_E_INVALID, "interaction_batch: max_path_len %d exceeds %d", ip->max_path_len, MPCX_MAX_PATH_LEN);
    const int fcap = max_rem / 4 - mpcx::SPARE_ROWS;
    const size_t lds = (size_t)max_rem * sizeof(double) + ((size_t)fcap * sizeof(unsigned short) + 7) / 8 * 8;
    mpcx::InterArgs ia{*ip, P, state, path_xyyaw, path_cs, path_off, path_len, prev_cut_len, ctx->pred,
                       obs_off, obs_cnt, obs_skip, traj_idx, hit_idx, hit_xy, cut_len, max_rem, fcap, x.prev_save,
                       x.bin_hint, x.bin_hint ? ctx->bins : nullptr, x.bin_hint ? ctx->bins + MPCX_ORDER_COPIES * MPCX_ORDER_BINS : nullptr,
                       x.key_prev, x.near, x.done, x.absent, n_obs_pool, x.prec, x.stand};
    if (x.prec) mpcx::launch_interaction_prec(P, lds, ctx->stream, ia);
    else if (x.absent) hipLaunchKernelGGL((mpcx::interaction_kernel<true, true>), dim3(P), dim3(64), lds, ctx->stream, ia);
    else if (x.done) hipLaunchKernelGGL(mpcx::interaction_kernel<true>, dim3(P), dim3(64), lds, ctx->stream, ia);
    else hipLaunchKernelGGL(mpcx::interaction_kernel<false>, dim3(P), dim3(64), lds, ctx->stream, ia);
    return mpcx_check_launch(ctx, "interaction kernels");
}

int32_t mpcx_ensure_pred(mpcx_ctx *ctx, size_t need) {
    return mpcx_grow(ctx, (void **)&ctx->pred, &ctx->pred_cap, need * sizeof(double), "the prediction scratch");
}

extern "C" int32_t mpcx_interaction_prediction(mpcx_ctx *ctx, int32_t rows, int32_t steps, double *out) {
    if (!ctx || !out || rows < 0 || steps < 1 || steps > MPCX_PRED_STEPS_MAX) return MPCX_E_INVALID;
    const size_t bytes = (size_t)rows * steps * 4 * sizeof(double);
    if (!ctx->pred || ctx->pred_cap < bytes)
        return mpcx_fail(ctx, MPCX_E_INVALID, "interaction_prediction: no prediction of %d rows x %d frames has been made on this context", rows, steps);
    if (rows == 0) return MPCX_OK;
    if (hipMemcpyAsync(out, ctx->pred, bytes, hipMemcpyDeviceToHost, ctx->stream) != hipSuccess || hipStreamSynchronize(ctx->stream) != hipSuccess)
        return mpcx_fail(ctx, MPCX_E_LAUNCH, "interaction_prediction: copy failed");
    return MPCX_OK;
}

extern "C" int32_t mpcx_moving_collision_batch(mpcx_ctx *ctx, const mpcx_interaction_params *ip, int32_t P,
                                               const double *ego_xyyaw, const double *ego_cs, const int32_t *ego_off,
                                               const int32_t *ego_len, const double *path_xyyaw, const double *path_cs,
                                               const int32_t *path_off, const int32_t *path_len,
                                               int32_t n_obs_pool, const double *obs_xyyaw, const double *obs_cs,
                                               const int32_t *obs_off, const int32_t *obs_cnt,
                                               int32_t *hit_idx, double *hit_xy) {
    if (!ctx) return MPCX_E_INVALID;
    if (P == 0) return MPCX_OK;
    if (!ip || P < 0 || n_obs_pool < 0 || !ego_xyyaw || !ego_cs || !ego_off || !ego_len || !path_xyyaw || !path_cs ||
        !path_off || !path_len || !obs_off || !obs_cnt || !hit_idx || !hit_xy || (n_obs_pool > 0 && (!obs_xyyaw || !obs_cs)))
        return mpcx_fail(ctx, MPCX_E_INVALID, "moving_collision_batch: null pointer or negative size");
    if (ip->pred_steps < 1 || ip->pred_steps > MPCX_PRED_STEPS_MAX || ip->frame_window < 0)
        return mpcx_fail(ctx, MPCX_E_INVALID, "moving_collision_batch: pred_steps outside 1..%d or negative frame_window", MPCX_PRED_STEPS_MAX);
    const size_t nposes = (size_t)n_obs_pool * ip->pred_steps;
    int32_t rc = mpcx_ensure_pred(ctx, (nposes ? nposes : 1) * 4);
    if (rc != MPCX_OK) return rc;
    if (nposes) {
        mpcx::PoseDiscArgs pd{*ip, (int)nposes, obs_xyyaw, obs_cs, ctx->pred};
        hipLaunchKernelGGL(mpcx::pose_disc_kernel, dim3((unsigned)((nposes + 255) / 256)), dim3(256), 0, ctx->stream, pd);
    }
    mpcx::MovArgs ma{*ip, P, ego_xyyaw, ego_cs, ego_off, ego_len, path_xyyaw, path_cs, path_off, path_len, ctx->pred,
                     obs_off, obs_cnt, hit_idx, hit_xy};
    hipLaunchKernelGGL(mpcx::moving_collision_kernel, dim3(P), dim3(64), 0, ctx->stream, ma);
    return mpcx_check_launch(ctx, "moving collision kernels");
}
#endif
```

mpc_for_av_at_intersection_amd/csrc/mpcx_loop.hip:

```cpp
#include "mpcx_common.h"
#include <cmath>
#include <cstring>

namespace mpcx {

struct PackArgs {
    int P;
    const double *state, *applied;
    double *obs6;
};

__global__ __launch_bounds__(256) void pack_pool_kernel(PackArgs a) {
    const int q = blockIdx.x * blockDim.x + threadIdx.x;
    if (q >= a.P) return;
    double *o = a.obs6 + 6 * (size_t)q;
    const double *s = a.state + 4 * (size_t)q;
    o[0] = s[0]; o[1] = s[1]; o[2] = s[2]; o[3] = s[3];
    o[4] = a.applied[2 * q + 1];
    o[5] = a.applied[2 * q];
}

}

static int32_t mpcx_loop_check_rows(mpcx_ctx *ctx, int32_t P, const int32_t *ego_row, int32_t pool_rows, const char *who = "closed_loop_run") {
    std::vector<int32_t> rows((size_t)P);
    if (hipMemcpy(rows.data(), ego_row, rows.size() * sizeof(int32_t), hipMemcpyDeviceToHost) != hipSuccess)
        return mpcx_fail(ctx, MPCX_E_LAUNCH, "%s: cannot read the agents' pool rows back for their check", who);
    for (int32_t q = 0; q < P; q++)
        if (rows[q] < 0 || rows[q] >= pool_rows)
            return mpcx_fail(ctx, MPCX_E_INVALID, "%s: agent %d sits in pool row %d of %d", who, q, rows[q], pool_rows);
    return MPCX_OK;
}

static int32_t *near_hints(const mpcx_ctx *ctx, int32_t P) { return ctx->prev_cut + P; }

static int32_t enqueue_step(mpcx_ctx *ctx, const mpcx_interaction_params *ip, const mpcx_closed_loop *c, const mpcx_run_log *log,
                            const mpcx_closed_loop_opts *o, const mpcx_retire *r, const mpcx_scene *sc, const mpcx_admit *ad,
                            const mpcx_respawn *rs, const mpcx_routes *rt, const mpcx_precedence *pc, const mpcx_signals *sg,
                            const mpcx_actuation *av) {
    const int P = c->P;
    const int32_t *done = r ? r->done : nullptr;
    int32_t *queue_len = r ? ctx->ticket + MPCX_TICKET_QUEUE_LEN : nullptr;
    const bool speed = o->stop_mode == MPCX_STOP_SPEED;
    ctx->bins_clean = false;
    int32_t rc, pool_rows = P;
    if (ad) {
        const int32_t na = c->n_actors > 0 ? c->n_actors : 0;
        rc = mpcx_admit_enqueue(ctx, ip, P, c->state, c->obs_off, c->obs_cnt, c->obs_skip, r->done, sc->n_rows, sc->absent, na, c->actors,
                                c->actor_state, c->tape, c->tape_rows, c->actor_row, ad);
        if (rc != MPCX_OK) return rc;
        if (pc && pc->mode == MPCX_PRECEDENCE_ENTRY) {
            rc = mpcx_precedence_enqueue(ctx, P, c->obs_off, c->obs_skip, ad, pc);
            if (rc != MPCX_OK) return rc;
        }
    }
    rc = mpcx_rollout_fork(ctx, P, c->state, c->u_sol, c->xbar, done);
    if (rc != MPCX_OK) return rc;
    const bool binned = P < (1 << 24);
    mpcx_interaction_extras ix;
    ix.prev_save = ctx->prev_cut;
    ix.near = near_hints(ctx, P);
    ix.bin_hint = binned ? c->iters : nullptr;
    ix.done = done;
    ix.absent = sc ? sc->absent : nullptr;
    if (pc) { ix.prec = pc->prec; ix.stand = pc->stand; }
    if (speed) ix.key_prev = c->cut_len;
    if (c->exchange == MPCX_SHARD_AGENTS) {
        mpcx::PackArgs pa{P, c->state, c->applied, c->obs_local};
        hipLaunchKernelGGL(mpcx::pack_pool_kernel, dim3((P + 63) / 64), dim3(64), 0, ctx->stream, pa);
        rc = mpcx_allgather_states(ctx, MPCX_SHARD_AGENTS, c->n_inst, c->agents_local, c->obs_local, c->obs6);
        if (rc != MPCX_OK) return rc;
        pool_rows = P * ctx->comm_world;
    } else {
        ix.pack_state = c->state; ix.pack_applied = c->applied;
        if (c->n_actors > 0) {
            rc = mpcx_traffic_enqueue(ctx, c->n_actors, c->actors, c->actor_state, c->tape, c->tape_rows, c->actor_row, c->pool_rows, c->obs6);
            if (rc != MPCX_OK) return rc;
            ix.ego_row = c->ego_row; ix.actor_row = c->actor_row;
            ix.n_ego = P; ix.n_actors = c->n_actors;
            pool_rows = c->pool_rows;
        }
    }
    rc = mpcx_interaction_enqueue(ctx, ip, P, c->state, c->path_xyyaw, c->path_cs, c->path_off, c->path_len,
                                  speed ? o->prev_len : c->cut_len , pool_rows, c->obs6,
                                  c->obs_off, c->obs_cnt, c->obs_skip, c->traj_idx, c->hit_idx, c->hit_xy, c->cut_len, ix);
    if (rc != MPCX_OK) return rc;
    if (sg) {
        rc = av ? mpcx_actuated_enqueue(ctx, P, c->dl, c->state, c->path_off, c->path_len, c->traj_idx, c->cut_len, done, sg, av)
                : mpcx_signal_enqueue(ctx, P, c->dl, c->state, c->path_off, c->path_len, c->traj_idx, c->cut_len, done, sg);
        if (rc != MPCX_OK) return rc;
    }
    const int Wd = ctx->mpc.T + 1;
    for (int pass = 0; pass < ctx->lin_passes; pass++) {
        const bool first = pass == 0;
        mpcx_window_extras wx{binned && first, near_hints(ctx, P), c->traj_idx, first};
        if (speed) { wx.stop_idx = c->cut_len; wx.v_ref = o->v_ref; wx.len_seen = o->prev_len; }
        wx.done = done; wx.queue_len = queue_len;
        rc = mpcx_window_enqueue(ctx, P, c->state, c->u_sol, c->path_xyyaw, c->path_v, c->path_off, speed ? c->path_len : c->cut_len, c->dl,
                                 c->target_ind, pass ? c->x_sol + 2 * Wd : nullptr, 4 * (int64_t)Wd, c->xref, c->reaches_end, c->xbar, wx);
        if (rc != MPCX_OK) return rc;
        const mpcx_qp_order ord{binned && first, c->iters, c->cut_len, ctx->prev_cut, queue_len};
        rc = mpcx_qp_enqueue(ctx, P, c->state, c->xref, c->xbar, c->reaches_end, c->u_sol, c->x_sol, c->u_sol, c->status, c->iters, c->kkt, ord);
        if (rc != MPCX_OK) return rc;
    }
    const mpcx_plant_extras px{c->iters, binned, done};
    rc = mpcx_plant_enqueue(ctx, P, c->state, c->u_sol, c->status, c->applied, px);
    if (rc == MPCX_OK) ctx->bins_clean = binned;
    if (rc != MPCX_OK) return rc;
    if (log) {
        rc = mpcx_record_enqueue(ctx, ip, P, c->state, c->applied, c->x_sol, c->path_xyyaw, c->path_off, c->path_len, c->target_ind, c->cut_len,
                                 c->traj_idx, c->hit_idx, c->status, c->iters, pool_rows, c->obs6, c->obs_off, c->obs_cnt, c->obs_skip, log,
                                 speed ? c->path_len : nullptr, done, sc ? sc->absent : nullptr);
        if (rc != MPCX_OK) return rc;
    }
    if (r) rc = mpcx_retire_enqueue(ctx, P, c->state, c->applied, c->path_xyyaw, c->path_off, c->path_len, c->target_ind,
                                    speed ? c->path_len : c->cut_len, r, sc, c->obs_skip);
    if (rc != MPCX_OK) return rc;
    if (rs && rt)
        rc = mpcx_route_enqueue(ctx, P, c->state, c->applied, c->u_sol, c->traj_idx, c->target_ind, c->cut_len, c->iters,
                                speed ? o->prev_len : nullptr, c->obs_skip, sc->n_rows, log, r, ad, rs, rt);
    else if (rs)
        rc = mpcx_respawn_enqueue(ctx, P, c->state, c->applied, c->u_sol, c->traj_idx, c->target_ind, c->cut_len, c->iters,
                                  speed ? o->prev_len : nullptr, c->obs_skip, sc->n_rows, log, r, ad, rs);
    return rc;
}

static int32_t closed_loop_run(mpcx_ctx *ctx, const mpcx_interaction_params *ip, const mpcx_closed_loop *c, const mpcx_run_log *log,
                               const mpcx_closed_loop_opts *opts, const mpcx_retire *retire, const mpcx_scene *scene, const mpcx_admit *admit,
                               const mpcx_respawn *respawn, const mpcx_routes *routes, const mpcx_precedence *precedence,
                               const mpcx_signals *signals, const mpcx_actuation *actuation, int32_t n_steps, int32_t use_graph) {
    if (!ctx) return MPCX_E_INVALID;
    if (!ctx->have_mpc) return mpcx_fail(ctx, MPCX_E_INVALID, "mpcx_set_mpc_params has not been called");
    if (!ip || !c || n_steps < 0 || c->P < 0) return mpcx_fail(ctx, MPCX_E_INVALID, "closed_loop_run: null descriptor or negative count");
    mpcx_closed_loop_opts opt = {};
    if (opts && opts->stop_mode != MPCX_STOP_CUT) {
        if (opts->stop_mode != MPCX_STOP_SPEED)
            return mpcx_fail(ctx, MPCX_E_INVALID, "closed_loop_run: unknown stop mode %d (MPCX_STOP_CUT or MPCX_STOP_SPEED)", opts->stop_mode);
        if (!std::isfinite(opts->v_ref)) return mpcx_fail(ctx, MPCX_E_INVALID, "closed_loop_run: MPCX_STOP_SPEED with a speed reference v_ref that is not finite");
        if (!opts->prev_len) return mpcx_fail(ctx, MPCX_E_INVALID, "closed_loop_run: MPCX_STOP_SPEED needs prev_len (P zero-initialised int32)");
        opt.stop_mode = MPCX_STOP_SPEED; opt.v_ref = opts->v_ref; opt.prev_len = opts->prev_len;
    }
    if (mpcx_record_absent(log)) log = nullptr;
    if (log) {
        const int32_t lrc = mpcx_record_validate(ctx, log, c->obs_skip);
        if (lrc != MPCX_OK) return lrc;
    }
    if (mpcx_retire_absent(retire)) retire = nullptr;
    if (retire) {
        const int32_t rrc = mpcx_retire_validate(ctx, retire, c->P);
        if (rrc != MPCX_OK) return rrc;
    }
    if (mpcx_scene_absent(scene)) scene = nullptr;
    if (scene) {
        const bool traffic = c->n_actors > 0;
        const size_t rows = traffic ? (size_t)(c->pool_rows > 0 ? c->pool_rows : 0) : (size_t)c->P;
        int32_t src = mpcx_scene_validate(ctx, scene, retire, c->exchange, rows, c->obs_skip);
        if (src == MPCX_OK && c->P > 0) src = mpcx_loop_check_rows(ctx, c->P, c->obs_skip, scene->n_rows, "scene");
        if (src != MPCX_OK) return src;
    }
    if (mpcx_admit_absent(admit)) admit = nullptr;
    if (admit) {
        const int32_t arc = mpcx_admit_validate(ctx, admit, retire, scene, c->exchange);
        if (arc != MPCX_OK) return arc;
    }
    if (mpcx_respawn_absent(respawn)) respawn = nullptr;
    if (respawn) {
        const int32_t prc = mpcx_respawn_validate(ctx, respawn, admit);
        if (prc != MPCX_OK) return prc;
    }
    if (mpcx_routes_absent(routes)) routes = nullptr;
    if (routes) {
        int32_t cap = ip->max_path_len > 0 ? ip->max_path_len : MPCX_MAX_REMAINING;
        if (cap < 512) cap = 512;
        cap = (cap + 63) / 64 * 64;
        const int32_t trc = mpcx_routes_validate(ctx, routes, respawn, c->path_off, c->path_len, cap);
        if (trc != MPCX_OK) return trc;
    }
    if (mpcx_precedence_absent(precedence)) precedence = nullptr;
    if (precedence) {
        const int32_t prc = mpcx_precedence_validate(ctx, precedence, scene, admit);
        if (prc != MPCX_OK) return prc;
    }
    if (mpcx_signals_absent(signals)) signals = nullptr;
    if (mpcx_actuation_absent(actuation)) actuation = nullptr;
    mpcx_actuation act;
    memset(&act, 0, sizeof act);
    if (actuation) {
        const int32_t arc = mpcx_actuation_validate(ctx, actuation, signals, c->P, c->exchange);
        if (arc != MPCX_OK) return arc;
        act.phase_groups = actuation->phase_groups; act.phase_time = actuation->phase_time; act.ctrl_time = actuation->ctrl_time;
        act.ctrl_of = actuation->ctrl_of; act.jstate = actuation->jstate; act.lights = actuation->lights; act.calls = actuation->calls;
        act.n_per = actuation->n_per; act.n_junctions = actuation->n_junctions; act.n_phases = actuation->n_phases;
        act.n_ctrl = actuation->n_ctrl;
        actuation = &act;
    } else if (signals) {
        const int32_t grc = mpcx_signals_validate(ctx, signals, c->exchange);
        if (grc != MPCX_OK) return grc;
    }
    if (n_steps == 0 || c->P == 0) return MPCX_OK;
    if (!c->state || !c->applied || !c->obs6 || !c->path_xyyaw || !c->path_cs || !c->path_off || !c->path_len ||
        !c->obs_off || !c->obs_cnt || !c->traj_idx || !c->target_ind || !c->hit_idx || !c->cut_len || !c->hit_xy ||
        !c->xref || !c->xbar || !c->reaches_end || !c->x_sol || !c->u_sol || !c->status || !c->iters || !c->kkt || !(c->dl > 0))
        return mpcx_fail(ctx, MPCX_E_INVALID, "closed_loop_run: null buffer in the descriptor or dl <= 0");
    if (ip->pred_steps < 1 || ip->pred_steps > MPCX_PRED_STEPS_MAX)
        return mpcx_fail(ctx, MPCX_E_INVALID, "closed_loop_run: pred_steps outside 1..%d", MPCX_PRED_STEPS_MAX);
    if (c->exchange != 0 && c->exchange != MPCX_SHARD_AGENTS)
        return mpcx_fail(ctx, MPCX_E_INVALID, "closed_loop_run: exchange must be 0 or MPCX_SHARD_AGENTS");
    if (c->exchange == MPCX_SHARD_AGENTS) {
        if (!c->obs_local || c->n_inst < 0 || c->agents_local < 0 || (long)c->n_inst * c->agents_local != (long)c->P)
            return mpcx_fail(ctx, MPCX_E_INVALID, "closed_loop_run: agent-sharded layout needs obs_local and P = n_inst * agents_local");
        if (use_graph) return mpcx_fail(ctx, MPCX_E_INVALID, "closed_loop_run: the agent-sharded layout (RCCL exchange) is not captured into a graph");
    }
    if (c->n_actors < 0) return mpcx_fail(ctx, MPCX_E_INVALID, "closed_loop_run: negative number of scripted actors");
    if (c->n_actors > 0) {
        if (c->exchange == MPCX_SHARD_AGENTS)
            return mpcx_fail(ctx, MPCX_E_INVALID, "closed_loop_run: scripted traffic is not supported in the agent-sharded layout (it is instance-local: shard by instances)");
        if (!c->actors || !c->actor_state || !c->actor_row || !c->ego_row || c->tape_rows < 0 || (long)c->pool_rows < (long)c->P + c->n_actors)
            return mpcx_fail(ctx, MPCX_E_INVALID, "closed_loop_run: scripted traffic needs actors, actor_state, actor_row, ego_row and pool_rows >= P + n_actors");
    }
    const size_t pool_rows = c->n_actors > 0 ? (size_t)c->pool_rows : (size_t)c->P * (c->exchange == MPCX_SHARD_AGENTS ? (size_t)ctx->comm_world : 1);
    int32_t rc = mpcx_ensure_pred(ctx, pool_rows * ip->pred_steps * 4);
    if (rc != MPCX_OK) return rc;
    if (c->n_actors > 0) {
        rc = mpcx_traffic_validate(ctx, c->n_actors, c->actors, c->tape, c->tape_rows, c->actor_row, c->pool_rows);
        if (rc != MPCX_OK) return rc;
        rc = mpcx_loop_check_rows(ctx, c->P, c->ego_row, c->pool_rows);
        if (rc != MPCX_OK) return rc;
    }
    rc = mpcx_ensure_ticket(ctx);
    if (rc != MPCX_OK) return rc;
    if (admit) {
        rc = mpcx_admit_prepare(ctx, (size_t)scene->n_rows);
        if (rc != MPCX_OK) return rc;
    }
    {
        const size_t slots = ((size_t)c->P + 63) / 64;
        if (slots > ctx->stats_slots) {
            int64_t keep[4] = {0, 0, 0, 0};
            if (ctx->stats) { rc = mpcx_closed_loop_stats(ctx, keep, 0); if (rc != MPCX_OK) return rc; (void)hipFree(ctx->stats); ctx->stats = nullptr; ctx->stats_slots = 0; }
            if (hipMalloc((void **)&ctx->stats, 4 * slots * sizeof(unsigned long long)) != hipSuccess ||
                hipMemsetAsync(ctx->stats, 0, 4 * slots * sizeof(unsigned long long), ctx->stream) != hipSuccess ||
                hipMemcpyAsync(ctx->stats, keep, sizeof keep, hipMemcpyHostToDevice, ctx->stream) != hipSuccess ||
                hipStreamSynchronize(ctx->stream) != hipSuccess)
                return mpcx_fail(ctx, MPCX_E_LAUNCH, "closed_loop_run: cannot allocate the run statistics");
            ctx->stats_slots = slots;
        }
    }
    rc = mpcx_ensure_order(ctx, (size_t)c->P);
    if (rc != MPCX_OK) return rc;
    {
        const size_t need = (size_t)MPCX_ORDER_COPIES * MPCX_ORDER_BINS + (size_t)c->P;
        if (need * sizeof(int32_t) > ctx->bins_cap) ctx->bins_clean = false;
        rc = mpcx_grow(ctx, (void **)&ctx->bins, &ctx->bins_cap, need * sizeof(int32_t), "the queue bins");
        if (rc != MPCX_OK) return rc;
        if (!ctx->bins_clean) {
            if (hipMemsetAsync(ctx->bins, 0, (size_t)MPCX_ORDER_COPIES * MPCX_ORDER_BINS * sizeof(int32_t), ctx->stream) != hipSuccess ||
                hipMemsetAsync(ctx->ticket, 0, MPCX_TICKET_WORDS * sizeof(int32_t), ctx->stream) != hipSuccess)
                return mpcx_fail(ctx, MPCX_E_LAUNCH, "closed_loop_run: hipMemsetAsync failed");
            ctx->bins_clean = true;
        }
    }
    rc = mpcx_grow(ctx, (void **)&ctx->prev_cut, &ctx->prev_cut_cap, 4 * (size_t)c->P * sizeof(int32_t), "the previous cut lengths");
    if (rc != MPCX_OK) return rc;

    if (!use_graph) {
        for (int s = 0; s < n_steps; s++) {
            rc = enqueue_step(ctx, ip, c, log, &opt, retire, scene, admit, respawn, routes, precedence, signals, actuation);
            if (rc != MPCX_OK) return rc;
        }
        return MPCX_OK;
    }

    if (!ctx->stream) return mpcx_fail(ctx, MPCX_E_INVALID, "closed_loop_run: graph replay needs a non-default stream");
    if (ctx->prof_qp)
        return mpcx_fail(ctx, MPCX_E_INVALID, "closed_loop_run: mpcx_profile_qp is on; the QP launches of a replayed graph are not bracketed by events -- run without graph or switch the hook off");
    unsigned char key[sizeof ctx->loop_key];
    static_assert(sizeof(mpcx_closed_loop) + sizeof(mpcx_run_log) + sizeof(mpcx_closed_loop_opts) + sizeof(mpcx_retire) + sizeof(mpcx_scene) + sizeof(mpcx_admit) + sizeof(mpcx_respawn) + sizeof(mpcx_routes) + sizeof(mpcx_precedence) + sizeof(mpcx_signals) + sizeof(mpcx_actuation) + sizeof(mpcx_interaction_params) +
                  sizeof(mpcx_mpc_params) + 10 * sizeof(void *) <= sizeof key,
                  "loop_key too small");
    memset(key, 0, sizeof key);
    size_t o = 0;
    memcpy(key + o, c, sizeof *c); o += sizeof *c;
    if (log) memcpy(key + o, log, sizeof *log);
    o += sizeof *log;
    memcpy(key + o, &opt, sizeof opt); o += sizeof opt;
    if (retire) memcpy(key + o, retire, sizeof *retire);
    o += sizeof *retire;
    if (scene) memcpy(key + o, scene, sizeof *scene);
    o += sizeof *scene;
    if (admit) memcpy(key + o, admit, sizeof *admit);
    o += sizeof *admit;
    if (respawn) memcpy(key + o, respawn, sizeof *respawn);
    o += sizeof *respawn;
    if (routes) memcpy(key + o, routes, sizeof *routes);
    o += sizeof *routes;
    if (precedence) memcpy(key + o, precedence, sizeof *precedence);
    o += sizeof *precedence;
    if (signals) memcpy(key + o, signals, sizeof *signals);
    o += sizeof *signals;
    if (actuation) memcpy(key + o, actuation, sizeof *actuation);
    o += sizeof *actuation;
    memcpy(key + o, &ctx->admit_tab, sizeof ctx->admit_tab); o += sizeof ctx->admit_tab;
    memcpy(key + o, ip, sizeof *ip); o += sizeof *ip;
    memcpy(key + o, &ctx->mpc, sizeof ctx->mpc); o += sizeof ctx->mpc;
    memcpy(key + o, &ctx->pred, sizeof ctx->pred); o += sizeof ctx->pred;
    memcpy(key + o, &ctx->tune, sizeof ctx->tune); o += sizeof ctx->tune;
    memcpy(key + o, &ctx->order, sizeof ctx->order); o += sizeof ctx->order;
    memcpy(key + o, &ctx->prev_cut, sizeof ctx->prev_cut); o += sizeof ctx->prev_cut;
    memcpy(key + o, &ctx->bins, sizeof ctx->bins); o += sizeof ctx->bins;
    memcpy(key + o, &ctx->qp_solver, sizeof ctx->qp_solver); o += sizeof ctx->qp_solver;
    memcpy(key + o, &ctx->lin_passes, sizeof ctx->lin_passes); o += sizeof ctx->lin_passes;
    memcpy(key + o, &ctx->stats, sizeof ctx->stats);
    if (!ctx->loop_exec || memcmp(key, ctx->loop_key, sizeof key) != 0) {
        if (ctx->loop_exec) {
            (void)hipStreamSynchronize(ctx->stream);
            (void)hipGraphExecDestroy(ctx->loop_exec);
            ctx->loop_exec = nullptr;
        }
        hipGraph_t graph = nullptr;
        if (hipStreamBeginCapture(ctx->stream, hipStreamCaptureModeThreadLocal) != hipSuccess)
            return mpcx_fail(ctx, MPCX_E_LAUNCH, "closed_loop_run: hipStreamBeginCapture failed");
        rc = enqueue_step(ctx, ip, c, log, &opt, retire, scene, admit, respawn, routes, precedence, signals, actuation);
        hipError_t e = hipStreamEndCapture(ctx->stream, &graph);
        if (rc != MPCX_OK) { if (graph) (void)hipGraphDestroy(graph); return rc; }
        if (e != hipSuccess || !graph) return mpcx_fail(ctx, MPCX_E_LAUNCH, "closed_loop_run: stream capture failed: %s", hipGetErrorString(e));
        e = hipGraphInstantiate(&ctx->loop_exec, graph, nullptr, nullptr, 0);
        (void)hipGraphDestroy(graph);
        if (e != hipSuccess) { ctx->loop_exec = nullptr; return mpcx_fail(ctx, MPCX_E_LAUNCH, "closed_loop_run: hipGraphInstantiate: %s", hipGetErrorString(e)); }
        memcpy(ctx->loop_key, key, sizeof key);
    }
    for (int s = 0; s < n_steps; s++)
        if (hipGraphLaunch(ctx->loop_exec, ctx->stream) != hipSuccess)
            return mpcx_fail(ctx, MPCX_E_LAUNCH, "closed_loop_run: hipGraphLaunch failed");
    return MPCX_OK;
}

extern "C" int32_t mpcx_closed_loop_run(mpcx_ctx *ctx, const mpcx_interaction_params *ip, const mpcx_closed_loop *c,
                                        int32_t n_steps, int32_t use_graph) {
    return closed_loop_run(ctx, ip, c, nullptr, nullptr, nullptr, nullptr, nullptr, nullptr, nullptr, nullptr, nullptr, nullptr, n_steps, use_graph);
}

extern "C" int32_t mpcx_closed_loop_run_logged(mpcx_ctx *ctx, const mpcx_interaction_params *ip, const mpcx_closed_loop *c,
                                               const mpcx_run_log *log, int32_t n_steps, int32_t use_graph) {
    return closed_loop_run(ctx, ip, c, log, nullptr, nullptr, nullptr, nullptr, nullptr, nullptr, nullptr, nullptr, nullptr, n_steps, use_graph);
}

extern "C" int32_t mpcx_closed_loop_run_opts(mpcx_ctx *ctx, const mpcx_interaction_params *ip, const mpcx_closed_loop *c,
                                             const mpcx_run_log *log, const mpcx_closed_loop_opts *opts, int32_t n_steps, int32_t use_graph) {
    return closed_loop_run(ctx, ip, c, log, opts, nullptr, nullptr, nullptr, nullptr, nullptr, nullptr, nullptr, nullptr, n_steps, use_graph);
}

extern "C" int32_t mpcx_closed_loop_run_retire(mpcx_ctx *ctx, const mpcx_interaction_params *ip, const mpcx_closed_loop *c,
                                               const mpcx_run_log *log, const mpcx_closed_loop_opts *opts, const mpcx_retire *retire,
                                               int32_t n_steps, int32_t use_graph) {
    return closed_loop_run(ctx, ip, c, log, opts, retire, nullptr, nullptr, nullptr, nullptr, nullptr, nullptr, nullptr, n_steps, use_graph);
}

extern "C" int32_t mpcx_closed_loop_run_scene(mpcx_ctx *ctx, const mpcx_interaction_params *ip, const mpcx_closed_loop *c,
                                              const mpcx_run_log *log, const mpcx_closed_loop_opts *opts, const mpcx_retire *retire,
                                              const mpcx_scene *scene, int32_t n_steps, int32_t use_graph) {
    return closed_loop_run(ctx, ip, c, log, opts, retire, scene, nullptr, nullptr, nullptr, nullptr, nullptr, nullptr, n_steps, use_graph);
}

extern "C" int32_t mpcx_closed_loop_run_admit(mpcx_ctx *ctx, const mpcx_interaction_params *ip, const mpcx_closed_loop *c,
                                              const mpcx_run_log *log, const mpcx_closed_loop_opts *opts, const mpcx_retire *retire,
                                              const mpcx_scene *scene, const mpcx_admit *admit, int32_t n_steps, int32_t use_graph) {
    return closed_loop_run(ctx, ip, c, log, opts, retire, scene, admit, nullptr, nullptr, nullptr, nullptr, nullptr, n_steps, use_graph);
}

extern "C" int32_t mpcx_closed_loop_run_respawn(mpcx_ctx *ctx, const mpcx_interaction_params *ip, const mpcx_closed_loop *c,
                                                const mpcx_run_log *log, const mpcx_closed_loop_opts *opts, const mpcx_retire *retire,
                                                const mpcx_scene *scene, const mpcx_admit *admit, const mpcx_respawn *respawn,
                                                int32_t n_steps, int32_t use_graph) {
    return mpcx_closed_loop_run_routes(ctx, ip, c, log, opts, retire, scene, admit, respawn, nullptr, n_steps, use_graph);
}

extern "C" int32_t mpcx_closed_loop_run_routes(mpcx_ctx *ctx, const mpcx_interaction_params *ip, const mpcx_closed_loop *c,
                                               const mpcx_run_log *log, const mpcx_closed_loop_opts *opts, const mpcx_retire *retire,
                                               const mpcx_scene *scene, const mpcx_admit *admit, const mpcx_respawn *respawn,
                                               const mpcx_routes *routes, int32_t n_steps, int32_t use_graph) {
    return mpcx_closed_loop_run_precedence(ctx, ip, c, log, opts, retire, scene, admit, respawn, routes, nullptr, n_steps, use_graph);
}

extern "C" int32_t mpcx_closed_loop_run_precedence(mpcx_ctx *ctx, const mpcx_interaction_params *ip, const mpcx_closed_loop *c,
                                                   const mpcx_run_log *log, const mpcx_closed_loop_opts *opts, const mpcx_retire *retire,
                                                   const mpcx_scene *scene, const mpcx_admit *admit, const mpcx_respawn *respawn,
                                                   const mpcx_routes *routes, const mpcx_precedence *precedence, int32_t n_steps,
                                                   int32_t use_graph) {
    return mpcx_closed_loop_run_signals(ctx, ip, c, log, opts, retire, scene, admit, respawn, routes, precedence, nullptr, n_steps, use_graph);
}

extern "C" int32_t mpcx_closed_loop_run_signals(mpcx_ctx *ctx, const mpcx_interaction_params *ip, const mpcx_closed_loop *c,
                                                const mpcx_run_log *log, const mpcx_closed_loop_opts *opts, const mpcx_retire *retire,
                                                const mpcx_scene *scene, const mpcx_admit *admit, const mpcx_respawn *respawn,
                                                const mpcx_routes *routes, const mpcx_precedence *precedence, const mpcx_signals *signals,
                                                int32_t n_steps, int32_t use_graph) {
    return mpcx_closed_loop_run_actuated(ctx, ip, c, log, opts, retire, scene, admit, respawn, routes, precedence, signals, nullptr, n_steps, use_graph);
}

extern "C" int32_t mpcx_closed_loop_run_actuated(mpcx_ctx *ctx, const mpcx_interaction_params *ip, const mpcx_closed_loop *c,
                                                 const mpcx_run_log *log, const mpcx_closed_loop_opts *opts, const mpcx_retire *retire,
                                                 const mpcx_scene *scene, const mpcx_admit *admit, const mpcx_respawn *respawn,
                                                 const mpcx_routes *routes, const mpcx_precedence *precedence, const mpcx_signals *signals,
                                                 const mpcx_actuation *actuation, int32_t n_steps, int32_t use_graph) {
    return closed_loop_run(ctx, ip, c, log, opts, retire, scene, admit, respawn, routes, precedence, signals, actuation, n_steps, use_graph);
}
```

mpc_for_av_at_intersection_amd/csrc/mpcx_prepare.hip:

```cpp
#include "mpcx_common.h"
#include <cmath>

namespace mpcx {

struct RefArgs {
    mpcx_mpc_params p;
    int B;
    const double *state, *path, *path_v;
    const int32_t *path_off, *path_len;
    double dl;
    int32_t *target_ind;
    double *xref;
    uint8_t *re;
    const double *ov;
    long ov_stride;
    const int32_t *bin_cnt, *keyslot;
    int32_t *order;
    const int32_t *near, *near_tidx;
    const int32_t *stop_idx;
    double v_ref;
    int32_t *len_seen;
    const int32_t *done;
    int32_t *queue_len;
};

constexpr int PREP_WAVES = 4;
constexpr int WIN_AGENTS = 8;
static_assert(WIN_AGENTS <= WAVE, "one lane per agent in parts 1 and 2");
template <bool RETIRE>
__global__ __launch_bounds__(64 * PREP_WAVES) void ref_window_kernel(RefArgs a) {
    __shared__ int s_first[MPCX_ORDER_COPIES][MPCX_ORDER_BINS];
    const int lane = threadIdx.x & 63, wave = threadIdx.x >> 6;
    const int T = a.p.T, W = T + 1;
    const int b0 = ((int)blockIdx.x * PREP_WAVES + wave) * WIN_AGENTS;
    const int nag = a.B - b0 < WIN_AGENTS ? a.B - b0 : WIN_AGENTS;
    const bool own = lane < nag;
    const int b = own ? b0 + lane : 0;
    bool gone = !own;
    if constexpr (RETIRE) gone = gone || a.done[b] != 0;
    const int off = a.path_off[b], n = a.path_len[b];
    const double x = a.state[4 * b], y = a.state[4 * b + 1], v = a.state[4 * b + 2];
    const int start = a.target_ind[b];
    const int ks = a.order ? a.keyslot[b] : 0;
    const int hs = a.near ? a.near[3 * b] : -1, hm = a.near ? a.near[3 * b + 1] : -1, hl = a.near ? a.near[3 * b + 2] : -1;
    const int hint = a.near ? a.near_tidx[b] : -1;
    const int stop_at = a.stop_idx ? a.stop_idx[b] : MPCX_NO_STOP;
    if (a.order) {
        static_assert(MPCX_ORDER_BINS == 64, "one bin per lane");
        if (wave == 0) {
            int cnt[MPCX_ORDER_COPIES], c = 0;
#pragma unroll
            for (int q = 0; q < MPCX_ORDER_COPIES; q++) { cnt[q] = a.bin_cnt[q * MPCX_ORDER_BINS + lane]; c += cnt[q]; }
            int sfx = c;
#pragma unroll
            for (int d = 1; d < 64; d <<= 1) { const int o = __shfl_down(sfx, d); sfx += lane + d < 64 ? o : 0; }
            if constexpr (RETIRE) { if (blockIdx.x == 0 && lane == 0) *a.queue_len = sfx; }
            int first = sfx - c;
#pragma unroll
            for (int q = 0; q < MPCX_ORDER_COPIES; q++) { s_first[q][lane] = first; first += cnt[q]; }
        }
        __syncthreads();
        if (!gone)
            a.order[s_first[b % MPCX_ORDER_COPIES][(ks >> 24) & (MPCX_ORDER_BINS - 1)] + (ks & 0xFFFFFF)] = b;
    }
    int s = -1;
    bool scan = false;
    if (!gone) {
        if (hm >= 0 && start >= hs && hl >= start && hm < n) s = hint;
        else scan = !(start < 0 || n <= 0);
    }
    for (unsigned long long todo = __ballot(scan); todo; todo &= todo - 1) {
        const int i = __ffsll((long long)todo) - 1;
        const int r = nearest_index_in_direction(a.path + 3 * (size_t)__shfl(off, i), __shfl(n, i), __shfl(start, i), __shfl(x, i), __shfl(y, i), lane);
        s = lane == i ? r : s;
    }
    int stop = 0x7fffffff;
    if (!gone) {
        a.target_ind[b] = s;
        stop = stop_at == MPCX_NO_STOP ? stop : stop_at;
        if (a.stop_idx && a.len_seen) a.len_seen[b] = n;
    }
    const int G = 64 / W;
    const int g = lane / W, t = lane - g * W;
    for (int base = 0; base < nag; base += G) {
        const int i = base + g;
        const bool on = g < G && i < nag;
        const int from = on ? i : 0;
        const bool skip = __shfl((int)gone, from) != 0;
        const int si = __shfl(s, from), ni = __shfl(n, from), oi = __shfl(off, from), stopi = __shfl(stop, from);
        const double vi = __shfl(v, from);
        if (!on || skip) continue;
        const int bi = b0 + i;
        const double *path = a.path + 3 * (size_t)oi;
        const double *pv = a.path_v ? a.path_v + (size_t)oi : nullptr;
        double *xr = a.xref + (size_t)bi * 4 * W;
        uint8_t *re = a.re + (size_t)bi * W;
        if (si < 0) {
            xr[t] = 0; xr[W + t] = 0; xr[2 * W + t] = 0; xr[3 * W + t] = 0; re[t] = 0;
            continue;
        }
        const double ov = vi > 10.0 / 3.6 ? vi : 10.0 / 3.6;
        const double step = __dmul_rn(fabs(ov), a.p.dt);
        const double *ovp = a.ov ? a.ov + (size_t)bi * a.ov_stride : nullptr;
        double travel = ovp ? __dmul_rn(fabs(ovp[0]), a.p.dt) : step;
        for (int k = 1; k <= t; k++) travel = __dadd_rn(travel, ovp ? __dmul_rn(fabs(ovp[k]), a.p.dt) : step);
        long long idx = (long long)rint(__ddiv_rn(travel, a.dl)) + si;
        if (idx > ni - 1) idx = ni - 1;
        xr[0 * W + t] = path[3 * idx];
        xr[1 * W + t] = path[3 * idx + 1];
        xr[2 * W + t] = idx >= stopi ? 0.0 : (pv ? pv[idx] : a.v_ref);
        xr[3 * W + t] = path[3 * idx + 2];
        re[t] = (idx == ni - 1);
    }
}

__device__ __forceinline__ double plant_tan(const mpcx_mpc_params &p, double delta) {
    return tan(fmax(fmin(delta, p.max_steer), -p.max_steer));
}
__device__ __forceinline__ double plant_rate_xy(double v, double cs) {
#pragma clang fp contract(off)
    return v * cs;
}
__device__ __forceinline__ double plant_rate_th(const mpcx_mpc_params &p, double v, double tn) {
#pragma clang fp contract(off)
    return (v / p.L) * tn;
}
__device__ __forceinline__ double plant_euler(const mpcx_mpc_params &p, double acc, double rate) { return fma(rate, p.dt, acc); }
__device__ __forceinline__ double plant_speed(const mpcx_mpc_params &p, double v, double a) {
    return fmax(fmin(plant_euler(p, v, a), p.max_speed), p.min_speed);
}
__device__ __forceinline__ void plant_step(const mpcx_mpc_params &p, double &x, double &y, double &v, double &th,
                                           double a, double delta) {
    const double tn = plant_tan(p, delta);
    double s, c;
    sincos(th, &s, &c);
    x = plant_euler(p, x, plant_rate_xy(v, c));
    y = plant_euler(p, y, plant_rate_xy(v, s));
    th = plant_euler(p, th, plant_rate_th(p, v, tn));
    v = plant_speed(p, v, a);
}

struct RollArgs {
    mpcx_mpc_params p;
    int B;
    const double *state, *u_warm;
    double *xbar;
    const int32_t *done;
};

constexpr int ROLL_GROUP = 4, ROLL_BLOCK = 256, ROLL_AGENTS = ROLL_BLOCK / ROLL_GROUP;
static_assert(WAVE % ROLL_GROUP == 0 && ROLL_BLOCK % WAVE == 0, "whole groups per wavefront");
inline size_t rollout_lds(int T) { return ROLL_AGENTS * (4 * (size_t)(T + 1) + 1) * sizeof(double); }
template <bool RETIRE>
__global__ __launch_bounds__(ROLL_BLOCK) void rollout_kernel(RollArgs a) {
    constexpr int G = ROLL_GROUP;
    extern __shared__ double s_roll[];
    const int T = a.p.T, W = T + 1;
    const int RS = 4 * W + 1;
    auto s_x = [&](int row) -> double * { return s_roll + (size_t)row * RS; };
    const int b0 = (int)blockIdx.x * ROLL_AGENTS;
    const int n = a.B - b0 < ROLL_AGENTS ? a.B - b0 : ROLL_AGENTS;
    const int r = (int)threadIdx.x / G, j = (int)threadIdx.x % G;
    bool gone = r >= n;
    if constexpr (RETIRE) gone = gone || a.done[b0 + r] != 0;
    if (j == 0) s_x(r)[4 * W] = gone ? 1.0 : 0.0;
    if (!gone) {
        const int b = b0 + r;
        double x = a.state[4 * b], y = a.state[4 * b + 1], v = a.state[4 * b + 2], th = a.state[4 * b + 3];
        double *xb = s_x(r);
        if (j == 0) { xb[0] = x; xb[W] = y; xb[2 * W] = v; xb[3 * W] = th; }
        const double *oa = a.u_warm ? a.u_warm + (size_t)b * 2 * T : nullptr;
        const auto euler = [&](double acc, double rate) { return plant_euler(a.p, acc, rate); };
        const auto speed = [&](double vv, double acc) { return plant_speed(a.p, vv, acc); };
        for (int t0 = 0; t0 < T; t0 += G) {
            const int t = t0 + j;
            const bool in = t < T;
            const double ai = oa && in ? oa[t] : 0.0, di = oa && in ? oa[T + t] : 0.0;
            const double tn = plant_tan(a.p, di);
            const double v0 = v, th0 = th;
            const double vn = group_chain<G>(v, ai, j, speed);
            const double vt = group_prev<G>(vn, v0, j);
            const double thn = group_chain<G>(th, plant_rate_th(a.p, vt, tn), j, euler);
            const double tht = group_prev<G>(thn, th0, j);
            double s, c;
            sincos(tht, &s, &c);
            const double xn = group_chain<G>(x, plant_rate_xy(vt, c), j, euler);
            const double yn = group_chain<G>(y, plant_rate_xy(vt, s), j, euler);
            if (in) { xb[t + 1] = xn; xb[W + t + 1] = yn; xb[2 * W + t + 1] = vn; xb[3 * W + t + 1] = thn; }
        }
    }
    __syncthreads();
    double *out = a.xbar + (size_t)b0 * 4 * W;
    for (int i = threadIdx.x; i < n * 4 * W; i += ROLL_BLOCK) {
        const int row = i / (4 * W);
        if (!RETIRE || s_x(row)[4 * W] == 0.0) out[i] = s_x(row)[i - row * 4 * W];
    }
}


struct PlantArgs {
    mpcx_mpc_params p;
    int B;
    double *state;
    double *u;
    const int32_t *status;
    double *applied;
    const mpcx_qp_tuning *tune;
    const int32_t *iters;
    unsigned long long *stats;
    int has_stats;
    int32_t *zero_bins, *zero_ticket;
    const int32_t *done;
};

__global__ __launch_bounds__(256) void plant_kernel(PlantArgs a) {
    if (a.zero_bins && blockIdx.x == 0) {
        for (int i = threadIdx.x; i < MPCX_ORDER_COPIES * MPCX_ORDER_BINS; i += blockDim.x) a.zero_bins[i] = 0;
        if (threadIdx.x < MPCX_TICKET_WORDS) a.zero_ticket[threadIdx.x] = 0;
    }
    const int b = blockIdx.x * blockDim.x + threadIdx.x;
    const bool gone = a.done && b < a.B && a.done[b] != 0;
    if (a.has_stats) {
        const bool in = b < a.B && !gone;
        const int it = in ? a.iters[b] : 0;
        const int bad = (in && a.status[b] != MPCX_QP_OPTIMAL) ? 1 : 0;
        int s_it = it, s_bad = bad, s_n = in ? 1 : 0, s_mx = it;
#pragma unroll
        for (int d = 32; d >= 1; d >>= 1) {
            s_it += __shfl_xor(s_it, d, WAVE); s_bad += __shfl_xor(s_bad, d, WAVE); s_n += __shfl_xor(s_n, d, WAVE);
            const int o = __shfl_xor(s_mx, d, WAVE); s_mx = o > s_mx ? o : s_mx;
        }
        if ((threadIdx.x & 63) == 0) {
            unsigned long long *w = a.stats + 4 * (size_t)(b >> 6);
            w[0] += (unsigned long long)s_n; w[1] += (unsigned long long)s_it; w[2] += (unsigned long long)s_bad;
            if ((unsigned long long)s_mx > w[3]) w[3] = (unsigned long long)s_mx;
        }
    }
    if (b >= a.B || gone) return;
    const int T = a.p.T;
    double di = a.applied[2 * b], ai;
    const bool ok = !a.status || a.status[b] == MPCX_QP_OPTIMAL;
    if (ok) { di = a.u[(size_t)b * 2 * T + T]; ai = a.u[(size_t)b * 2 * T]; }
    else {
        ai = a.tune ? a.tune[b].max_decel : a.p.max_decel;
        for (int t = 0; t < 2 * T; t++) a.u[(size_t)b * 2 * T + t] = 0.0;
    }
    a.applied[2 * b] = di; a.applied[2 * b + 1] = ai;
    double x = a.state[4 * b], y = a.state[4 * b + 1], v = a.state[4 * b + 2], th = a.state[4 * b + 3];
    plant_step(a.p, x, y, v, th, ai, di);
    a.state[4 * b] = x; a.state[4 * b + 1] = y; a.state[4 * b + 2] = v; a.state[4 * b + 3] = th;
}

}

extern "C" int32_t mpcx_mpc_prepare_batch(mpcx_ctx *ctx, int32_t B, const double *state, const double *u_warm,
                                          const double *path_xyyaw, const double *path_v, const int32_t *path_off,
                                          const int32_t *path_len, double dl, int32_t *target_ind, double *xref, uint8_t *reaches_end, double *xbar) {
    return mpcx_mpc_prepare_batch_ov(ctx, B, state, u_warm, path_xyyaw, path_v, path_off, path_len, dl, target_ind, nullptr, 0, xref, reaches_end, xbar);
}

extern "C" int32_t mpcx_mpc_prepare_batch_ov(mpcx_ctx *ctx, int32_t B, const double *state, const double *u_warm,
                                             const double *path_xyyaw, const double *path_v, const int32_t *path_off,
                                             const int32_t *path_len, double dl, int32_t *target_ind, const double *ov, int64_t ov_stride,
                                             double *xref, uint8_t *reaches_end, double *xbar) {
    return mpcx_window_enqueue(ctx, B, state, u_warm, path_xyyaw, path_v, path_off, path_len, dl, target_ind, ov, ov_stride, xref, reaches_end, xbar, {});
}

extern "C" int32_t mpcx_mpc_prepare_batch_stop(mpcx_ctx *ctx, int32_t B, const double *state, const double *u_warm,
                                               const double *path_xyyaw, const double *path_v, const int32_t *path_off,
                                               const int32_t *path_len, double dl, int32_t *target_ind, const double *ov, int64_t ov_stride,
                                               const int32_t *stop_idx, double v_ref, int32_t *len_seen,
                                               double *xref, uint8_t *reaches_end, double *xbar) {
    mpcx_window_extras wx;
    wx.stop_idx = stop_idx; wx.v_ref = v_ref; wx.len_seen = len_seen;
    return mpcx_window_enqueue(ctx, B, state, u_warm, path_xyyaw, path_v, path_off, path_len, dl, target_ind, ov, ov_stride, xref, reaches_end, xbar, wx);
}

int32_t mpcx_window_enqueue(mpcx_ctx *ctx, int32_t B, const double *state, const double *u_warm, const double *path_xyyaw, const double *path_v,
                            const int32_t *path_off, const int32_t *path_len, double dl, int32_t *target_ind, const double *ov, int64_t ov_stride,
                            double *xref, uint8_t *reaches_end, double *xbar, const mpcx_window_extras &x) {
    if (!ctx) return MPCX_E_INVALID;
    if (!ctx->have_mpc) return mpcx_fail(ctx, MPCX_E_INVALID, "mpcx_set_mpc_params has not been called");
    if (B == 0) return MPCX_OK;
    if (B < 0 || !state || !path_xyyaw || !path_off || !path_len || !target_ind || !xref || !reaches_end || !xbar || !(dl > 0))
        return mpcx_fail(ctx, MPCX_E_INVALID, "mpc_prepare_batch: null pointer, negative batch or dl <= 0");
    if (ov && ov_stride < (int64_t)ctx->mpc.T + 1)
        return mpcx_fail(ctx, MPCX_E_INVALID, "mpc_prepare_batch_ov: ov_stride %lld is smaller than T + 1", (long long)ov_stride);
    if (x.stop_idx && !std::isfinite(x.v_ref))
        return mpcx_fail(ctx, MPCX_E_INVALID, "mpc_prepare_batch_stop: v_ref is not finite");
    mpcx::RefArgs ra{ctx->mpc, B, state, path_xyyaw, path_v, path_off, path_len, dl, target_ind, xref, reaches_end, ov, (long)ov_stride,
                     x.scatter ? ctx->bins : nullptr, x.scatter ? ctx->bins + MPCX_ORDER_COPIES * MPCX_ORDER_BINS : nullptr, x.scatter ? ctx->order : nullptr,
                     x.near, x.near ? x.tidx : nullptr, x.stop_idx, x.stop_idx ? x.v_ref : 0.0, x.stop_idx ? x.len_seen : nullptr,
                     x.done, x.queue_len};
    const bool retire = x.done != nullptr;
    if (retire && (!x.scatter || !x.queue_len))
        return mpcx_fail(ctx, MPCX_E_INVALID, "mpc_prepare_batch: retirement needs the queue order built beside the window selection");
    const bool forked = x.rollout_forked;
    if (!forked) {
        int32_t rc = mpcx_rollout_fork(ctx, B, state, u_warm, xbar, x.done);
        if (rc != MPCX_OK) return rc;
    }
    if (forked && hipStreamWaitEvent(ctx->stream, ctx->ev_join, 0) != hipSuccess)
        return mpcx_fail(ctx, MPCX_E_LAUNCH, "mpc_prepare_batch: cannot join the side stream");
    constexpr int per_block = mpcx::PREP_WAVES * mpcx::WIN_AGENTS;
    const dim3 wgrid((B + per_block - 1) / per_block), wblock(64 * mpcx::PREP_WAVES);
    if (retire) hipLaunchKernelGGL(mpcx::ref_window_kernel<true>, wgrid, wblock, 0, ctx->stream, ra);
    else hipLaunchKernelGGL(mpcx::ref_window_kernel<false>, wgrid, wblock, 0, ctx->stream, ra);
    if (!forked && hipStreamWaitEvent(ctx->stream, ctx->ev_join, 0) != hipSuccess)
        return mpcx_fail(ctx, MPCX_E_LAUNCH, "mpc_prepare_batch: cannot join the side stream");
    return mpcx_check_launch(ctx, "prepare kernels");
}

int32_t mpcx_rollout_fork(mpcx_ctx *ctx, int32_t B, const double *state, const double *u_warm, double *xbar, const int32_t *done) {
    mpcx::RollArgs ro{ctx->mpc, B, state, u_warm, xbar, done};
    if (hipEventRecord(ctx->ev_fork, ctx->stream) != hipSuccess || hipStreamWaitEvent(ctx->side, ctx->ev_fork, 0) != hipSuccess)
        return mpcx_fail(ctx, MPCX_E_LAUNCH, "mpc_prepare_batch: cannot fork the side stream");
    const size_t roll_lds = mpcx::rollout_lds(ctx->mpc.T);
    const dim3 rgrid((B + mpcx::ROLL_AGENTS - 1) / mpcx::ROLL_AGENTS), rblock(mpcx::ROLL_BLOCK);
    if (done) hipLaunchKernelGGL(mpcx::rollout_kernel<true>, rgrid, rblock, roll_lds, ctx->side, ro);
    else hipLaunchKernelGGL(mpcx::rollout_kernel<false>, rgrid, rblock, roll_lds, ctx->side, ro);
    const int32_t rc = mpcx_check_launch(ctx, "rollout_kernel");
    if (rc != MPCX_OK) return rc;
    if (hipEventRecord(ctx->ev_join, ctx->side) != hipSuccess)
        return mpcx_fail(ctx, MPCX_E_LAUNCH, "mpc_prepare_batch: cannot record the join event");
    return MPCX_OK;
}

extern "C" int32_t mpcx_plant_step_batch(mpcx_ctx *ctx, int32_t B, double *state, double *u,
                                         const int32_t *status, double *applied) {
    return mpcx_plant_enqueue(ctx, B, state, u, status, applied, {});
}

int32_t mpcx_plant_enqueue(mpcx_ctx *ctx, int32_t B, double *state, double *u, const int32_t *status, double *applied, const mpcx_plant_extras &x) {
    if (!ctx) return MPCX_E_INVALID;
    if (!ctx->have_mpc) return mpcx_fail(ctx, MPCX_E_INVALID, "mpcx_set_mpc_params has not been called");
    if (B == 0) return MPCX_OK;
    if (B < 0 || !state || !u || !applied) return mpcx_fail(ctx, MPCX_E_INVALID, "plant_step_batch: null pointer");
    if (ctx->tune && ctx->tune_rows != B)
        return mpcx_fail(ctx, MPCX_E_INVALID, "plant_step_batch: %d tuning rows are set but the batch has %d agents", ctx->tune_rows, B);
    const bool st = ctx->stats && x.stats_iters && status;
    const bool rz = x.reset_bins && ctx->bins && ctx->ticket;
    mpcx::PlantArgs pa{ctx->mpc, B, state, u, status, applied, ctx->tune, x.stats_iters, ctx->stats, st ? 1 : 0,
                       rz ? ctx->bins : nullptr, rz ? ctx->ticket : nullptr, x.done};
    hipLaunchKernelGGL(mpcx::plant_kernel, dim3((B + 63) / 64), dim3(64), 0, ctx->stream, pa);
    return mpcx_check_launch(ctx, "plant_kernel");
}

extern "C" int32_t mpcx_closed_loop_stats(mpcx_ctx *ctx, int64_t *out4, int32_t reset) {
    if (!ctx || !out4) return MPCX_E_INVALID;
    out4[0] = out4[1] = out4[2] = out4[3] = 0;
    if (!ctx->stats || !ctx->stats_slots) return MPCX_OK;
    std::vector<unsigned long long> h(4 * ctx->stats_slots);
    if (hipMemcpyAsync(h.data(), ctx->stats, h.size() * sizeof(unsigned long long), hipMemcpyDeviceToHost, ctx->stream) != hipSuccess ||
        hipStreamSynchronize(ctx->stream) != hipSuccess)
        return mpcx_fail(ctx, MPCX_E_LAUNCH, "closed_loop_stats: copy failed");
    for (size_t w = 0; w < ctx->stats_slots; w++) {
        out4[0] += (int64_t)h[4 * w]; out4[1] += (int64_t)h[4 * w + 1]; out4[2] += (int64_t)h[4 * w + 2];
        if ((int64_t)h[4 * w + 3] > out4[3]) out4[3] = (int64_t)h[4 * w + 3];
    }
    if (reset && hipMemsetAsync(ctx->stats, 0, h.size() * sizeof(unsigned long long), ctx->stream) != hipSuccess)
        return mpcx_fail(ctx, MPCX_E_LAUNCH, "closed_loop_stats: reset failed");
    return MPCX_OK;
}

extern "C" int32_t mpcx_closed_loop_queue(mpcx_ctx *ctx, int32_t P, int32_t *order, int32_t *keyslot) {
    if (!ctx || !order || !keyslot || P < 0) return MPCX_E_INVALID;
    const size_t counters = (size_t)MPCX_ORDER_COPIES * MPCX_ORDER_BINS;
    if (!ctx->order || !ctx->bins || ctx->order_cap < (size_t)P * sizeof(int32_t) || ctx->bins_cap < (counters + (size_t)P) * sizeof(int32_t))
        return mpcx_fail(ctx, MPCX_E_INVALID, "closed_loop_queue: no closed loop has built a work queue for %d agents on this context", P);
    if (P == 0) return MPCX_OK;
    if (hipMemcpyAsync(order, ctx->order, (size_t)P * sizeof(int32_t), hipMemcpyDeviceToHost, ctx->stream) != hipSuccess ||
        hipMemcpyAsync(keyslot, ctx->bins + counters, (size_t)P * sizeof(int32_t), hipMemcpyDeviceToHost, ctx->stream) != hipSuccess ||
        hipStreamSynchronize(ctx->stream) != hipSuccess)
        return mpcx_fail(ctx, MPCX_E_LAUNCH, "closed_loop_queue: copy failed");
    return MPCX_OK;
}
```

mpc_for_av_at_intersection_amd/runtime.py:

```python
import ctypes as C
import functools
from dataclasses import dataclass, field
from typing import Tuple, Optional, Sequence

import numpy as np
import torch

from . import _lib


@dataclass
class MpcParams:
    T: int = 13
    dt: float = 0.2
    L: float = 2.86
    w_perp: float = 20.0
    w_para: float = 1.0
    R: Sequence[float] = (0.01, 0.01)
    Rd: Sequence[float] = (0.01, 1.0)
    Q_v_yaw: Sequence[float] = (0.0, 0.5)
    Qf_base: Sequence[float] = (1.0, 1.0, 0.0, 0.5)
    R_end: Sequence[float] = (10.0, 10.0)
    max_speed: float = 30.0 / 3.6
    min_speed: float = -5.0
# ... 562 lines not shown
        elif log is None:
            self._chk(self.lib.mpcx_closed_loop_run(self._ctx, C.byref(cip), C.byref(desc), int(n_steps), 1 if graph else 0))
        else:
            self._chk(self.lib.mpcx_closed_loop_run_logged(self._ctx, C.byref(cip), C.byref(desc), C.byref(log), int(n_steps), 1 if graph else 0))

    @_ordered
    def signal_step(self, dl: float, state, path_off, path_len, traj_idx, cut_len, signals: '_lib.SignalsC', done=None):
        Pn = int(state.shape[0])
        self._want(state, torch.float64, (Pn, 4), 'state')
        for name, t in (('path_off', path_off), ('path_len', path_len), ('traj_idx', traj_idx), ('cut_len', cut_len)):
            self._want(t, torch.int32, (Pn,), name)
        if done is not None:
            self._want(done, torch.int32, (Pn,), 'done')
        self._chk(self.lib.mpcx_signal_step_batch(self._ctx, Pn, float(dl), _ptr(state), _ptr(path_off), _ptr(path_len), _ptr(traj_idx),
                                                  _ptr(cut_len), _ptr(done), C.byref(signals)))

    @_ordered
    def actuated_step(self, dl: float, state, path_off, path_len, traj_idx, cut_len, signals: '_lib.SignalsC', actuation: '_lib.ActuationC',
                      done=None):
        Pn = int(state.shape[0])
        self._want(state, torch.float64, (Pn, 4), 'state')
        for name, t in (('path_off', path_off), ('path_len', path_len), ('traj_idx', traj_idx), ('cut_len', cut_len)):
            self._want(t, torch.int32, (Pn,), name)
        if done is not None:
            self._want(done, torch.int32, (Pn,), 'done')
        self._chk(self.lib.mpcx_actuated_step_batch(self._ctx, Pn, float(dl), _ptr(state), _ptr(path_off), _ptr(path_len), _ptr(traj_idx),
                                                    _ptr(cut_len), _ptr(done), C.byref(signals), C.byref(actuation)))

    @_ordered
    def admit_step(self, ip: InteractionParams, state, obs_off, obs_cnt, obs_skip, done, absent, admit: '_lib.AdmitC', actors=None,
                   actor_state=None, actor_row=None, tape=None, precedence: Optional['_lib.PrecedenceC'] = None):
        Pn = int(state.shape[0])
        self._want(state, torch.float64, (Pn, 4), 'state'); self._want(done, torch.int32, (Pn,), 'done')
        self._want(absent, torch.int32, (absent.shape[0],), 'absent')
        for nm, t in (('obs_off', obs_off), ('obs_cnt', obs_cnt), ('obs_skip', obs_skip)):
            self._want(t, torch.int32, (Pn,), nm)
        n = 0
        if actor_state is not None:
            n = int(actor_state.shape[0])
            self._want(actors, torch.uint8, (n * _lib.TRAFFIC_ACTOR_DTYPE.itemsize,), 'actors')
            self._want(actor_state, torch.float64, (n, 4), 'actor_state'); self._want(actor_row, torch.int32, (n,), 'actor_row')
            if tape is not None:
                self._want(tape, torch.float64, (tape.shape[0], 6), 'tape')
        cip = ip.to_c()
        args = (self._ctx, C.byref(cip), Pn, _ptr(state), _ptr(obs_off), _ptr(obs_cnt), _ptr(obs_skip), _ptr(done),
                int(absent.shape[0]), _ptr(absent), n, _ptr(actors) if n else None,
                _ptr(actor_state) if n else None, _ptr(tape) if n else None,
                0 if (tape is None or not n) else int(tape.shape[0]), _ptr(actor_row) if n else None,
                C.byref(admit))
        if precedence is not None:
            self._chk(self.lib.mpcx_admit_step_batch_precedence(*args, C.byref(precedence)))
            return
        self._chk(self.lib.mpcx_admit_step_batch(*args))

    @_ordered
    def respawn_step(self, state, applied, u_sol, traj_idx, target_ind, cut_len, iters, obs_skip, n_obs_pool: int, retire: '_lib.RetireC',
                     admit: '_lib.AdmitC', respawn: '_lib.RespawnC', prev_len=None, log: Optional['_lib.RunLogC'] = None,
                     routes: Optional['_lib.RoutesC'] = None, max_path_len: int = 0):
        Pn = int(state.shape[0])
        self._want(state, torch.float64, (Pn, 4), 'state'); self._want(applied, torch.float64, (Pn, 2), 'applied')
        self._want(u_sol, torch.float64, (Pn, 2, self.params.T), 'u_sol')
        for nm, t in (('traj_idx', traj_idx), ('target_ind', target_ind), ('cut_len', cut_len), ('iters', iters), ('obs_skip', obs_skip)):
            self._want(t, torch.int32, (Pn,), nm)
        if prev_len is not None:
            self._want(prev_len, torch.int32, (Pn,), 'prev_len')
        if routes is not None:
            self._chk(self.lib.mpcx_respawn_step_batch_routes(self._ctx, Pn, _ptr(state), _ptr(applied), _ptr(u_sol), _ptr(traj_idx),
                                                              _ptr(target_ind), _ptr(cut_len), _ptr(iters), _ptr(prev_len), _ptr(obs_skip),
                                                              int(n_obs_pool), None if log is None else C.byref(log), C.byref(retire),
                                                              C.byref(admit), C.byref(respawn), C.byref(routes), int(max_path_len)))
            return
        self._chk(self.lib.mpcx_respawn_step_batch(self._ctx, Pn, _ptr(state), _ptr(applied), _ptr(u_sol), _ptr(traj_idx), _ptr(target_ind),
                                                   _ptr(cut_len), _ptr(iters), _ptr(prev_len), _ptr(obs_skip), int(n_obs_pool),
                                                   None if log is None else C.byref(log), C.byref(retire), C.byref(admit), C.byref(respawn)))

    @_ordered
    def episode_summary(self, A: int, R: int, served, ep_i32, ep_f64):
        Pn, G = int(ep_i32.shape[0]), int(ep_i32.shape[1])
        self._want(served, torch.int32, (Pn,), 'served'); self._want(ep_i32, torch.int32, (Pn, G, 8), 'ep_i32')
        self._want(ep_f64, torch.float64, (Pn, G, 2), 'ep_f64')
        if A < 1 or Pn % int(A):
            raise MpcxError('episode_summary: %d slots do not divide into instances of %d (MPCX_E_INVALID)' % (Pn, A))
        B = Pn // int(A)
        out_i = torch.zeros((B, int(R), 4), dtype=torch.int64, device=self.device)
        out_f = torch.full((B, int(R)), float('inf'), dtype=torch.float64, device=self.device)
        self._chk(self.lib.mpcx_episode_summary(self._ctx, Pn, int(A), G, int(R), _ptr(served), _ptr(ep_i32), _ptr(ep_f64), _ptr(out_i), _ptr(out_f)))
        return out_i, out_f

    @_ordered
    def record_step(self, ip: InteractionParams, state, applied, x_sol, path, path_off, path_len, target_ind, cut_len, traj_idx, hit_idx,
                    status, iters, obs6, obs_off, obs_cnt, obs_skip, log: '_lib.RunLogC', goal_len=None):
        Pn = int(state.shape[0])
        self._want(state, torch.float64, (Pn, 4), 'state'); self._want(applied, torch.float64, (Pn, 2), 'applied')
        self._want(x_sol, torch.float64, (Pn, 4, self.params.T + 1), 'x_sol'); self._want(obs6, torch.float64, (obs6.shape[0], 6), 'obs6')
        for nm, t in (('path_off', path_off), ('path_len', path_len), ('target_ind', target_ind), ('cut_len', cut_len), ('traj_idx', traj_idx),
                      ('hit_idx', hit_idx), ('status', status), ('iters', iters), ('obs_off', obs_off), ('obs_cnt', obs_cnt)):
            self._want(t, torch.int32, (Pn,), nm)
        if obs_skip is not None:
            self._want(obs_skip, torch.int32, (Pn,), 'obs_skip')
        cip = ip.to_c()
        if goal_len is not None:
            self._want(goal_len, torch.int32, (Pn,), 'goal_len')
            self._chk(self.lib.mpcx_record_step_batch_goal(self._ctx, C.byref(cip), Pn, _ptr(state), _ptr(applied), _ptr(x_sol), _ptr(path),
                                                           _ptr(path_off), _ptr(path_len), _ptr(target_ind), _ptr(cut_len), _ptr(traj_idx),
                                                           _ptr(hit_idx), _ptr(status), _ptr(iters), int(obs6.shape[0]), _ptr(obs6), _ptr(obs_off),
                                                           _ptr(obs_cnt), _ptr(obs_skip), _ptr(goal_len), C.byref(log)))
            return
        self._chk(self.lib.mpcx_record_step_batch(self._ctx, C.byref(cip), Pn, _ptr(state), _ptr(applied), _ptr(x_sol), _ptr(path), _ptr(path_off),
                                                  _ptr(path_len), _ptr(target_ind), _ptr(cut_len), _ptr(traj_idx), _ptr(hit_idx), _ptr(status),
                                                  _ptr(iters), int(obs6.shape[0]), _ptr(obs6), _ptr(obs_off), _ptr(obs_cnt), _ptr(obs_skip),
                                                  C.byref(log)))

    @_ordered
    def closed_loop_stats(self, reset: bool = True):
        out = (C.c_int64 * 4)()
        self._chk(self.lib.mpcx_closed_loop_stats(self._ctx, out, 1 if reset else 0))
        return dict(agent_steps=int(out[0]), iterations=int(out[1]), failures=int(out[2]), max_iterations=int(out[3]))

    def closed_loop_queue(self, P: int):
        order, keyslot = np.zeros(P, dtype=np.int32), np.zeros(P, dtype=np.int32)
        self._chk(self.lib.mpcx_closed_loop_queue(self._ctx, int(P), order.ctypes.data, keyslot.ctypes.data))
        return order, keyslot

    def interaction_prediction(self, rows: int, steps: int):
        out = np.zeros((int(rows), int(steps), 2, 2))
        self._chk(self.lib.mpcx_interaction_prediction(self._ctx, int(rows), int(steps), out.ctypes.data))
        return out

    @_ordered
    def set_instance_tuning(self, rows: Optional[torch.Tensor]):
        if rows is None:
            self._chk(self.lib.mpcx_set_instance_tuning(self._ctx, None, 0))
        else:
            self._want(rows, torch.float64, (rows.shape[0], 16), 'tuning rows')
            self._chk(self.lib.mpcx_set_instance_tuning(self._ctx, _ptr(rows), int(rows.shape[0])))
        self._tuning = rows

    @_ordered
    def set_qp_order_hint(self, prev_iters: Optional[torch.Tensor], ref_now: Optional[torch.Tensor] = None,
                          ref_prev: Optional[torch.Tensor] = None):
        for t in (prev_iters, ref_now, ref_prev):
            if t is not None:
                self._want(t, torch.int32, None, 'order hint')
        self._chk(self.lib.mpcx_qp_set_order_hint(self._ctx, _ptr(prev_iters), _ptr(ref_now), _ptr(ref_prev)))
        self._order_hint = (prev_iters, ref_now, ref_prev)

    def set_qp_solver(self, which: str):
        self._chk(self.lib.mpcx_set_qp_solver(self._ctx, {'auto': 0, 'condensed': 1, 'stage': 2}[which]))

    def set_linearisation_passes(self, passes: int):
        self._chk(self.lib.mpcx_set_linearisation_passes(self._ctx, int(passes)))
        self.lin_passes = int(passes)

    def profile_qp(self, enable: bool):
        self._chk(self.lib.mpcx_profile_qp(self._ctx, 1 if enable else 0))

    @_ordered
    def profile_qp_read(self):
        ms, n = C.c_double(0.0), C.c_int32(0)
        self._chk(self.lib.mpcx_profile_qp_read(self._ctx, C.byref(ms), C.byref(n)))
        return ms.value, n.value

    def comm_unique_id(self) -> bytes:
        buf = C.create_string_buffer(_lib.COMM_ID_BYTES)
        rc = self.lib.mpcx_comm_unique_id(buf)
        if rc != 0:
            raise MpcxError('mpcx_comm_unique_id failed (%d)' % rc)
        return buf.raw

    def comm_init(self, world: int, rank: int, unique_id: bytes):
        buf = C.create_string_buffer(bytes(unique_id), _lib.COMM_ID_BYTES)
        self._chk(self.lib.mpcx_comm_init(self._ctx, int(world), int(rank), buf))
        self.comm_world, self.comm_rank = int(world), int(rank)

    def comm_destroy(self):
        self._chk(self.lib.mpcx_comm_destroy(self._ctx))
        self.comm_world, self.comm_rank = 1, 0

    @_ordered
    def allgather_states(self, layout: int, local: torch.Tensor, out: torch.Tensor):
        n_inst, a_loc = int(local.shape[0]), int(local.shape[1])
        self._want(local, torch.float64, (n_inst, a_loc, 6), 'local'); self._want(out, torch.float64, None, 'out')
        world = getattr(self, 'comm_world', 1)
        if out.numel() != world * local.numel():
            raise MpcxError('allgather_states: out holds %d doubles, expected %d' % (out.numel(), world * local.numel()))
        self._chk(self.lib.mpcx_allgather_states(self._ctx, int(layout), n_inst, a_loc, _ptr(local), _ptr(out)))
        return out

    def synchronize(self):
        self.stream.synchronize()


class SearchModel:

    def __init__(self, ctx: Context, templates, last_pose, edge_cost, hp, hp_off):
        self.ctx = ctx
        tmpl_off = np.cumsum([0] + [len(t) for t in templates]).astype(np.int32)
        tmpl_xy = np.ascontiguousarray(np.concatenate([np.asarray(t)[:, :2] for t in templates]), np.float64)
        last_pose = np.ascontiguousarray(last_pose, np.float64)
        edge_cost = np.ascontiguousarray(edge_cost, np.float64)
        hp = np.ascontiguousarray(hp, np.float64).reshape(-1, 3)
        hp_off = np.ascontiguousarray(hp_off, np.int32)
        self.n_prim = len(templates)
        self.n_obst = len(hp_off) - 1
        self.n_pts_of = [len(t) for t in templates]
        self.n_rows = int(len(hp))
        self.edge_cost = edge_cost
        vp = C.c_void_p
        self._h = ctx.lib.mpcx_search_model_create(ctx._ctx, self.n_prim, vp(tmpl_off.ctypes.data), vp(tmpl_xy.ctypes.data),
                                                   vp(last_pose.ctypes.data), vp(edge_cost.ctypes.data), self.n_obst,
                                                   vp(hp_off.ctypes.data), vp(hp.ctypes.data))
        if not self._h:
            raise MpcxError('mpcx_search_model_create: %s' % ctx.lib.mpcx_last_error(ctx._ctx).decode())

    def close(self):
        if getattr(self, '_h', None):
            self.ctx.lib.mpcx_search_model_destroy(self._h)
            self._h = None

    def __del__(self):
        try:
            self.close()
        except Exception:
            pass
```

Baseline: 9.025 million.

## Fuse plant step, rollout and obstacle prediction into one head kernel per step

Adds a head kernel that runs the previous step's plant update, the warm-start rollout into xbar, and the obstacle prediction (one extra wavefront per workgroup) in a single launch. The closed loop uses it when no graph, exchange, actors or special modes are active. Interaction and window preparation then skip their own prediction and rollout launches. This removes several kernel launches and round trips through global memory per timestep, at the cost of a larger workgroup and a separate code path that must stay consistent with the unfused one.

Result: faster. 9.273 million (median of 6 runs) (+2.7%).

```diff
diff --git a/include/mpcx.h b/include/mpcx.h
--- a/include/mpcx.h
+++ b/include/mpcx.h
@@ -203,6 +203,7 @@
 } mpcx_closed_loop;
 int32_t mpcx_closed_loop_run(mpcx_ctx *ctx, const mpcx_interaction_params *ip, const mpcx_closed_loop *cl,
                              int32_t n_steps, int32_t use_graph);
+int32_t mpcx_set_step_fusion(mpcx_ctx *ctx, int32_t on);
 int32_t mpcx_closed_loop_stats(mpcx_ctx *ctx, int64_t *out4 , int32_t reset);
 int32_t mpcx_closed_loop_queue(mpcx_ctx *ctx, int32_t P, int32_t *order , int32_t *keyslot );
 int32_t mpcx_interaction_prediction(mpcx_ctx *ctx, int32_t rows, int32_t steps, double *out );
diff --git a/mpc_for_av_at_intersection_amd/_lib.py b/mpc_for_av_at_intersection_amd/_lib.py
--- a/mpc_for_av_at_intersection_amd/_lib.py
+++ b/mpc_for_av_at_intersection_amd/_lib.py
@@ -155,7 +155,7 @@
            'mpcx_transform_batch', 'mpcx_cutoff_index_batch', 'mpcx_predict_obstacles_batch', 'mpcx_selftest_wave_ops', 'mpcx_selftest_mfma',
            'mpcx_closed_loop_run', 'mpcx_profile_qp', 'mpcx_profile_qp_read', 'mpcx_set_instance_tuning', 'mpcx_set_qp_solver', 'mpcx_qp_set_order_hint', 'mpcx_expand_multi_batch',
            'mpcx_comm_unique_id', 'mpcx_comm_init', 'mpcx_comm_destroy', 'mpcx_allgather_states', 'mpcx_closed_loop_stats',
-           'mpcx_mpc_prepare_batch_ov', 'mpcx_set_linearisation_passes', 'mpcx_astar_batch', 'mpcx_traffic_step_batch',
+           'mpcx_mpc_prepare_batch_ov', 'mpcx_set_linearisation_passes', 'mpcx_set_step_fusion', 'mpcx_astar_batch', 'mpcx_traffic_step_batch',
            'mpcx_record_step_batch', 'mpcx_closed_loop_run_logged', 'mpcx_mpc_prepare_batch_stop', 'mpcx_record_step_batch_goal',
            'mpcx_closed_loop_run_opts', 'mpcx_closed_loop_run_retire', 'mpcx_closed_loop_run_scene', 'mpcx_closed_loop_run_admit',
            'mpcx_admit_step_batch', 'mpcx_closed_loop_run_respawn', 'mpcx_respawn_step_batch', 'mpcx_closed_loop_run_routes',
@@ -185,6 +185,7 @@
     lib.mpcx_mpc_prepare_batch_ov.restype = i32
     lib.mpcx_mpc_prepare_batch_ov.argtypes = [vp, i32, vp, vp, vp, vp, vp, vp, C.c_double, vp, vp, C.c_int64, vp, vp, vp]
     lib.mpcx_set_linearisation_passes.restype = i32; lib.mpcx_set_linearisation_passes.argtypes = [vp, i32]
+    lib.mpcx_set_step_fusion.restype = i32; lib.mpcx_set_step_fusion.argtypes = [vp, i32]
     lib.mpcx_astar_batch.restype = i32
     lib.mpcx_astar_batch.argtypes = [vp, i32, vp, vp, i32, vp, vp, i32, vp, vp, vp]
     lib.mpcx_search_model_create.restype = vp
diff --git a/mpc_for_av_at_intersection_amd/csrc/mpcx_api.hip b/mpc_for_av_at_intersection_amd/csrc/mpcx_api.hip
--- a/mpc_for_av_at_intersection_amd/csrc/mpcx_api.hip
+++ b/mpc_for_av_at_intersection_amd/csrc/mpcx_api.hip
@@ -119,6 +119,12 @@
     return MPCX_OK;
 }
 
+int32_t mpcx_set_step_fusion(mpcx_ctx *ctx, int32_t on) {
+    if (!ctx) return MPCX_E_INVALID;
+    ctx->step_fusion = on != 0;
+    return MPCX_OK;
+}
+
 int32_t mpcx_profile_qp(mpcx_ctx *ctx, int32_t enable) {
     if (!ctx) return MPCX_E_INVALID;
     ctx->prof_qp = enable != 0;
diff --git a/mpc_for_av_at_intersection_amd/csrc/mpcx_common.h b/mpc_for_av_at_intersection_amd/csrc/mpcx_common.h
--- a/mpc_for_av_at_intersection_amd/csrc/mpcx_common.h
+++ b/mpc_for_av_at_intersection_amd/csrc/mpcx_common.h
@@ -34,6 +34,7 @@
     void *multi = nullptr;
     size_t multi_cap = 0;
     int qp_solver = 0;
+    bool step_fusion = true;
     int lin_passes = 1;
     bool prof_qp = false;
     std::vector<hipEvent_t> prof_ev;
@@ -51,6 +52,7 @@
 
 struct mpcx_interaction_extras {
     const double *pack_state = nullptr, *pack_applied = nullptr;
+    bool predicted = false;
     const int32_t *ego_row = nullptr, *actor_row = nullptr;
     int32_t n_ego = 0, n_actors = 0;
     int32_t *prev_save = nullptr;
@@ -66,6 +68,7 @@
     bool scatter = false;
     const int32_t *near = nullptr, *tidx = nullptr;
     bool rollout_forked = false;
+    bool rollout_done = false;
     const int32_t *stop_idx = nullptr;
     double v_ref = 0.0;
     int32_t *len_seen = nullptr;
@@ -92,6 +95,8 @@
 int32_t mpcx_qp_enqueue(mpcx_ctx *ctx, int32_t B, const double *x0, const double *xref, const double *xbar, const uint8_t *reaches_end,
                       const double *u_warm, double *x_out, double *u_out, int32_t *status, int32_t *iters, double *kkt, const mpcx_qp_order &ord);
 int32_t mpcx_plant_enqueue(mpcx_ctx *ctx, int32_t B, double *state, double *u, const int32_t *status, double *applied, const mpcx_plant_extras &x);
+int32_t mpcx_head_enqueue(mpcx_ctx *ctx, const mpcx_interaction_params *ip, int32_t P, double *state, double *applied, double *u,
+                          const int32_t *status, const int32_t *iters, double *xbar, double *obs6, bool plant, bool reset_bins);
 
 int32_t mpcx_fail(mpcx_ctx *ctx, int32_t code, const char *fmt, ...);
 int32_t mpcx_check_launch(mpcx_ctx *ctx, const char *what);
diff --git a/mpc_for_av_at_intersection_amd/csrc/mpcx_interaction.hip b/mpc_for_av_at_intersection_amd/csrc/mpcx_interaction.hip
--- a/mpc_for_av_at_intersection_amd/csrc/mpcx_interaction.hip
+++ b/mpc_for_av_at_intersection_amd/csrc/mpcx_interaction.hip
@@ -1,4 +1,5 @@
 #include "mpcx_common.h"
+#include "mpcx_predict_core.h"
 
 namespace mpcx {
 
@@ -7,11 +8,6 @@
 #else
 constexpr bool FORCE_EXACT = false;
 #endif
-
-__device__ __forceinline__ void pose_discs(const mpcx_interaction_params &ip, double px, double py, double c, double s, double *out) {
-#pragma unroll
-    for (int d = 0; d < 2; d++) disc_centre(px, py, c, s, ip.circle_centers[2 * d], ip.circle_centers[2 * d + 1], out[2 * d], out[2 * d + 1]);
-}
 
 struct PredArgs {
     mpcx_interaction_params ip;
@@ -48,20 +44,7 @@
         x = s6[0]; y = s6[1]; v = s6[2]; yaw = s6[3]; acc = s6[4]; steer = s6[5];
     }
     if constexpr (SCENE) { if (a.absent[o] != 0) return; }
-    const double tn = tan(steer);
-    const double dt = a.ip.dt;
-    double s, c;
-    sincos(yaw, &s, &c);
-    if constexpr (STAND) pose_discs(a.ip, x, y, c, s, a.stand + 4 * (size_t)o);
-    double *out = a.pred + (size_t)o * a.ip.pred_steps * 4;
-    for (int k = 0; k < a.ip.pred_steps; k++) {
-        x = __dadd_rn(x, __dmul_rn(__dmul_rn(v, c), dt));
-        y = __dadd_rn(y, __dmul_rn(__dmul_rn(v, s), dt));
-        v = __dadd_rn(v, __dmul_rn(acc, dt));
-        yaw = __dadd_rn(yaw, __dmul_rn(__dmul_rn(__ddiv_rn(v, a.ip.L), tn), dt));
-        sincos(yaw, &s, &c);
-        pose_discs(a.ip, x, y, c, s, out + 4 * k);
-    }
+    predict_row<STAND>(a.ip, x, y, v, yaw, acc, steer, STAND ? a.stand + 4 * (size_t)o : nullptr, a.pred + (size_t)o * a.ip.pred_steps * 4);
 }
 
 struct InterArgs {
@@ -800,7 +783,8 @@
     if (x.absent && (!x.done || n_obs_pool < 1)) return mpcx_fail(ctx, MPCX_E_INVALID, "interaction_batch: a scene without retirement or without a pool");
     if ((x.prec || x.stand) && (!x.absent || !x.prec || !x.stand)) return mpcx_fail(ctx, MPCX_E_INVALID, "interaction_batch: precedence without a scene, or without one of prec and stand");
     { int32_t rc = mpcx_ensure_pred(ctx, (size_t)(n_obs_pool > 0 ? n_obs_pool : 1) * ip->pred_steps * 4); if (rc != MPCX_OK) return rc; }
-    if (n_obs_pool > 0 && x.pack_state && x.ego_row) {
+    if (x.predicted) {
+    } else if (n_obs_pool > 0 && x.pack_state && x.ego_row) {
         const int lanes = x.n_ego + x.n_actors;
         mpcx::PredArgs pa{*ip, lanes, n_obs_pool, obs6, ctx->pred, x.pack_state, x.pack_applied, const_cast<double *>(obs6),
                           x.ego_row, x.actor_row, x.n_ego, x.absent, x.stand};
diff --git a/mpc_for_av_at_intersection_amd/csrc/mpcx_loop.hip b/mpc_for_av_at_intersection_amd/csrc/mpcx_loop.hip
--- a/mpc_for_av_at_intersection_amd/csrc/mpcx_loop.hip
+++ b/mpc_for_av_at_intersection_amd/csrc/mpcx_loop.hip
@@ -122,6 +122,43 @@
     else if (rs)
         rc = mpcx_respawn_enqueue(ctx, P, c->state, c->applied, c->u_sol, c->traj_idx, c->target_ind, c->cut_len, c->iters,
                                   speed ? o->prev_len : nullptr, c->obs_skip, sc->n_rows, log, r, ad, rs);
+    return rc;
+}
+
+static int32_t enqueue_fused_run(mpcx_ctx *ctx, const mpcx_interaction_params *ip, const mpcx_closed_loop *c, const mpcx_closed_loop_opts *o,
+                                 int32_t n_steps) {
+    const int P = c->P;
+    const bool speed = o->stop_mode == MPCX_STOP_SPEED;
+    const bool binned = P < (1 << 24);
+    int32_t rc;
+    for (int s = 0; s < n_steps; s++) {
+        ctx->bins_clean = false;
+        rc = mpcx_head_enqueue(ctx, ip, P, c->state, c->applied, c->u_sol, c->status, c->iters, c->xbar, c->obs6, s > 0, binned);
+        if (rc != MPCX_OK) return rc;
+        mpcx_interaction_extras ix;
+        ix.prev_save = ctx->prev_cut;
+        ix.near = near_hints(ctx, P);
+        ix.bin_hint = binned ? c->iters : nullptr;
+        if (speed) ix.key_prev = c->cut_len;
+        ix.pack_state = c->state; ix.pack_applied = c->applied;
+        ix.predicted = true;
+        rc = mpcx_interaction_enqueue(ctx, ip, P, c->state, c->path_xyyaw, c->path_cs, c->path_off, c->path_len,
+                                      speed ? o->prev_len : c->cut_len, P, c->obs6, c->obs_off, c->obs_cnt, c->obs_skip, c->traj_idx, c->hit_idx,
+                                      c->hit_xy, c->cut_len, ix);
+        if (rc != MPCX_OK) return rc;
+        mpcx_window_extras wx{binned, near_hints(ctx, P), c->traj_idx, true};
+        wx.rollout_done = true;
+        if (speed) { wx.stop_idx = c->cut_len; wx.v_ref = o->v_ref; wx.len_seen = o->prev_len; }
+        rc = mpcx_window_enqueue(ctx, P, c->state, c->u_sol, c->path_xyyaw, c->path_v, c->path_off, speed ? c->path_len : c->cut_len, c->dl,
+                                 c->target_ind, nullptr, 4 * (int64_t)(ctx->mpc.T + 1), c->xref, c->reaches_end, c->xbar, wx);
+        if (rc != MPCX_OK) return rc;
+        const mpcx_qp_order ord{binned, c->iters, c->cut_len, ctx->prev_cut, nullptr};
+        rc = mpcx_qp_enqueue(ctx, P, c->state, c->xref, c->xbar, c->reaches_end, c->u_sol, c->x_sol, c->u_sol, c->status, c->iters, c->kkt, ord);
+        if (rc != MPCX_OK) return rc;
+    }
+    const mpcx_plant_extras px{c->iters, binned, nullptr};
+    rc = mpcx_plant_enqueue(ctx, P, c->state, c->u_sol, c->status, c->applied, px);
+    if (rc == MPCX_OK) ctx->bins_clean = binned;
     return rc;
 }
 
@@ -264,6 +301,9 @@
     if (rc != MPCX_OK) return rc;
 
     if (!use_graph) {
+        if (ctx->step_fusion && c->exchange == 0 && c->n_actors == 0 && ctx->lin_passes == 1 && !log && !retire && !scene && !admit && !respawn &&
+            !routes && !precedence && !signals && !actuation)
+            return enqueue_fused_run(ctx, ip, c, &opt, n_steps);
         for (int s = 0; s < n_steps; s++) {
             rc = enqueue_step(ctx, ip, c, log, &opt, retire, scene, admit, respawn, routes, precedence, signals, actuation);
             if (rc != MPCX_OK) return rc;
diff --git a/mpc_for_av_at_intersection_amd/csrc/mpcx_predict_core.h b/mpc_for_av_at_intersection_amd/csrc/mpcx_predict_core.h
--- /dev/null
+++ b/mpc_for_av_at_intersection_amd/csrc/mpcx_predict_core.h
@@ -0,0 +1,29 @@
+#pragma once
+#include "mpcx_common.h"
+
+namespace mpcx {
+
+__device__ __forceinline__ void pose_discs(const mpcx_interaction_params &ip, double px, double py, double c, double s, double *out) {
+#pragma unroll
+    for (int d = 0; d < 2; d++) disc_centre(px, py, c, s, ip.circle_centers[2 * d], ip.circle_centers[2 * d + 1], out[2 * d], out[2 * d + 1]);
+}
+
+template <bool STAND>
+__device__ __forceinline__ void predict_row(const mpcx_interaction_params &ip, double x, double y, double v, double yaw, double acc,
+                                            double steer, double *stand, double *out) {
+    const double tn = tan(steer);
+    const double dt = ip.dt;
+    double s, c;
+    sincos(yaw, &s, &c);
+    if constexpr (STAND) pose_discs(ip, x, y, c, s, stand);
+    for (int k = 0; k < ip.pred_steps; k++) {
+        x = __dadd_rn(x, __dmul_rn(__dmul_rn(v, c), dt));
+        y = __dadd_rn(y, __dmul_rn(__dmul_rn(v, s), dt));
+        v = __dadd_rn(v, __dmul_rn(acc, dt));
+        yaw = __dadd_rn(yaw, __dmul_rn(__dmul_rn(__ddiv_rn(v, ip.L), tn), dt));
+        sincos(yaw, &s, &c);
+        pose_discs(ip, x, y, c, s, out + 4 * k);
+    }
+}
+
+}
diff --git a/mpc_for_av_at_intersection_amd/csrc/mpcx_prepare.hip b/mpc_for_av_at_intersection_amd/csrc/mpcx_prepare.hip
--- a/mpc_for_av_at_intersection_amd/csrc/mpcx_prepare.hip
+++ b/mpc_for_av_at_intersection_amd/csrc/mpcx_prepare.hip
@@ -1,4 +1,5 @@
 #include "mpcx_common.h"
+#include "mpcx_predict_core.h"
 #include <cmath>
 
 namespace mpcx {
@@ -151,6 +152,29 @@
 constexpr int ROLL_GROUP = 4, ROLL_BLOCK = 256, ROLL_AGENTS = ROLL_BLOCK / ROLL_GROUP;
 static_assert(WAVE % ROLL_GROUP == 0 && ROLL_BLOCK % WAVE == 0, "whole groups per wavefront");
 inline size_t rollout_lds(int T) { return ROLL_AGENTS * (4 * (size_t)(T + 1) + 1) * sizeof(double); }
+__device__ __forceinline__ void rollout_group(const mpcx_mpc_params &p, double x, double y, double v, double th, const double *oa, int j, double *xb) {
+    constexpr int G = ROLL_GROUP;
+    const int T = p.T, W = T + 1;
+    if (j == 0) { xb[0] = x; xb[W] = y; xb[2 * W] = v; xb[3 * W] = th; }
+    const auto euler = [&](double acc, double rate) { return plant_euler(p, acc, rate); };
+    const auto speed = [&](double vv, double acc) { return plant_speed(p, vv, acc); };
+    for (int t0 = 0; t0 < T; t0 += G) {
+        const int t = t0 + j;
+        const bool in = t < T;
+        const double ai = oa && in ? oa[t] : 0.0, di = oa && in ? oa[T + t] : 0.0;
+        const double tn = plant_tan(p, di);
+        const double v0 = v, th0 = th;
+        const double vn = group_chain<G>(v, ai, j, speed);
+        const double vt = group_prev<G>(vn, v0, j);
+        const double thn = group_chain<G>(th, plant_rate_th(p, vt, tn), j, euler);
+        const double tht = group_prev<G>(thn, th0, j);
+        double s, c;
+        sincos(tht, &s, &c);
+        const double xn = group_chain<G>(x, plant_rate_xy(vt, c), j, euler);
+        const double yn = group_chain<G>(y, plant_rate_xy(vt, s), j, euler);
+        if (in) { xb[t + 1] = xn; xb[W + t + 1] = yn; xb[2 * W + t + 1] = vn; xb[3 * W + t + 1] = thn; }
+    }
+}
 template <bool RETIRE>
 __global__ __launch_bounds__(ROLL_BLOCK) void rollout_kernel(RollArgs a) {
     constexpr int G = ROLL_GROUP;
@@ -167,27 +191,7 @@
     if (!gone) {
         const int b = b0 + r;
         double x = a.state[4 * b], y = a.state[4 * b + 1], v = a.state[4 * b + 2], th = a.state[4 * b + 3];
-        double *xb = s_x(r);
-        if (j == 0) { xb[0] = x; xb[W] = y; xb[2 * W] = v; xb[3 * W] = th; }
-        const double *oa = a.u_warm ? a.u_warm + (size_t)b * 2 * T : nullptr;
-        const auto euler = [&](double acc, double rate) { return plant_euler(a.p, acc, rate); };
-        const auto speed = [&](double vv, double acc) { return plant_speed(a.p, vv, acc); };
-        for (int t0 = 0; t0 < T; t0 += G) {
-            const int t = t0 + j;
-            const bool in = t < T;
-            const double ai = oa && in ? oa[t] : 0.0, di = oa && in ? oa[T + t] : 0.0;
-            const double tn = plant_tan(a.p, di);
-            const double v0 = v, th0 = th;
-            const double vn = group_chain<G>(v, ai, j, speed);
-            const double vt = group_prev<G>(vn, v0, j);
-            const double thn = group_chain<G>(th, plant_rate_th(a.p, vt, tn), j, euler);
-            const double tht = group_prev<G>(thn, th0, j);
-            double s, c;
-            sincos(tht, &s, &c);
-            const double xn = group_chain<G>(x, plant_rate_xy(vt, c), j, euler);
-            const double yn = group_chain<G>(y, plant_rate_xy(vt, s), j, euler);
-            if (in) { xb[t + 1] = xn; xb[W + t + 1] = yn; xb[2 * W + t + 1] = vn; xb[3 * W + t + 1] = thn; }
-        }
+        rollout_group(a.p, x, y, v, th, a.u_warm ? a.u_warm + (size_t)b * 2 * T : nullptr, j, s_x(r));
     }
     __syncthreads();
     double *out = a.xbar + (size_t)b0 * 4 * W;
@@ -213,6 +217,20 @@
     const int32_t *done;
 };
 
+__device__ __forceinline__ void plant_stats(unsigned long long *stats, int b, bool in, int it, bool bad) {
+    int s_it = it, s_bad = bad ? 1 : 0, s_n = in ? 1 : 0, s_mx = it;
+#pragma unroll
+    for (int d = 32; d >= 1; d >>= 1) {
+        s_it += __shfl_xor(s_it, d, WAVE); s_bad += __shfl_xor(s_bad, d, WAVE); s_n += __shfl_xor(s_n, d, WAVE);
+        const int o = __shfl_xor(s_mx, d, WAVE); s_mx = o > s_mx ? o : s_mx;
+    }
+    if ((threadIdx.x & 63) == 0) {
+        unsigned long long *w = stats + 4 * (size_t)(b >> 6);
+        w[0] += (unsigned long long)s_n; w[1] += (unsigned long long)s_it; w[2] += (unsigned long long)s_bad;
+        if ((unsigned long long)s_mx > w[3]) w[3] = (unsigned long long)s_mx;
+    }
+}
+
 __global__ __launch_bounds__(256) void plant_kernel(PlantArgs a) {
     if (a.zero_bins && blockIdx.x == 0) {
         for (int i = threadIdx.x; i < MPCX_ORDER_COPIES * MPCX_ORDER_BINS; i += blockDim.x) a.zero_bins[i] = 0;
@@ -222,19 +240,7 @@
     const bool gone = a.done && b < a.B && a.done[b] != 0;
     if (a.has_stats) {
         const bool in = b < a.B && !gone;
-        const int it = in ? a.iters[b] : 0;
-        const int bad = (in && a.status[b] != MPCX_QP_OPTIMAL) ? 1 : 0;
-        int s_it = it, s_bad = bad, s_n = in ? 1 : 0, s_mx = it;
-#pragma unroll
-        for (int d = 32; d >= 1; d >>= 1) {
-            s_it += __shfl_xor(s_it, d, WAVE); s_bad += __shfl_xor(s_bad, d, WAVE); s_n += __shfl_xor(s_n, d, WAVE);
-            const int o = __shfl_xor(s_mx, d, WAVE); s_mx = o > s_mx ? o : s_mx;
-        }
-        if ((threadIdx.x & 63) == 0) {
-            unsigned long long *w = a.stats + 4 * (size_t)(b >> 6);
-            w[0] += (unsigned long long)s_n; w[1] += (unsigned long long)s_it; w[2] += (unsigned long long)s_bad;
-            if ((unsigned long long)s_mx > w[3]) w[3] = (unsigned long long)s_mx;
-        }
+        plant_stats(a.stats, b, in, in ? a.iters[b] : 0, in && a.status[b] != MPCX_QP_OPTIMAL);
     }
     if (b >= a.B || gone) return;
     const int T = a.p.T;
@@ -249,6 +255,80 @@
     double x = a.state[4 * b], y = a.state[4 * b + 1], v = a.state[4 * b + 2], th = a.state[4 * b + 3];
     plant_step(a.p, x, y, v, th, ai, di);
     a.state[4 * b] = x; a.state[4 * b + 1] = y; a.state[4 * b + 2] = v; a.state[4 * b + 3] = th;
+}
+
+struct HeadArgs {
+    mpcx_mpc_params p;
+    mpcx_interaction_params ip;
+    int B;
+    double *state, *applied, *u;
+    double *xbar, *obs6, *pred;
+    const int32_t *status, *iters;
+    const mpcx_qp_tuning *tune;
+    unsigned long long *stats;
+    int32_t *zero_bins, *zero_ticket;
+};
+
+constexpr int HEAD_BLOCK = ROLL_BLOCK + WAVE;
+static_assert(ROLL_AGENTS == WAVE, "the prediction wavefront holds the workgroup's agents one per lane; its statistics slot is plant_kernel's");
+template <bool PLANT>
+__global__ __launch_bounds__(HEAD_BLOCK) void head_kernel(HeadArgs a) {
+    constexpr int G = ROLL_GROUP;
+    extern __shared__ double s_roll[];
+    const int T = a.p.T, W = T + 1;
+    const int RS = 4 * W + 1;
+    const int tid = (int)threadIdx.x;
+    const bool pred_wave = tid >= ROLL_BLOCK;
+    const int b0 = (int)blockIdx.x * ROLL_AGENTS;
+    const int n = a.B - b0 < ROLL_AGENTS ? a.B - b0 : ROLL_AGENTS;
+    const int r = pred_wave ? tid - ROLL_BLOCK : tid / G, j = tid % G;
+    const bool in = r < n;
+    const int b = b0 + (in ? r : 0);
+    double x = a.state[4 * b], y = a.state[4 * b + 1], v = a.state[4 * b + 2], th = a.state[4 * b + 3];
+    double di = 0.0, ai = 0.0;
+    bool failed = false;
+    if constexpr (PLANT) {
+        if (a.zero_bins && blockIdx.x == 0) {
+            for (int i = tid; i < MPCX_ORDER_COPIES * MPCX_ORDER_BINS; i += HEAD_BLOCK) a.zero_bins[i] = 0;
+            if (tid < MPCX_TICKET_WORDS) a.zero_ticket[tid] = 0;
+        }
+        failed = a.status[b] != MPCX_QP_OPTIMAL;
+        const int it = pred_wave && in ? a.iters[b] : 0;
+        di = a.applied[2 * b];
+        if (!failed) { di = a.u[(size_t)b * 2 * T + T]; ai = a.u[(size_t)b * 2 * T]; }
+        else { ai = a.p.max_decel; if (a.tune) ai = a.tune[b].max_decel; }
+        plant_step(a.p, x, y, v, th, ai, di);
+        __syncthreads();
+        if (pred_wave) {
+            plant_stats(a.stats, b0 + r, in, it, in && failed);
+            if (in) {
+                if (failed) for (int t = 0; t < 2 * T; t++) a.u[(size_t)b * 2 * T + t] = 0.0;
+                a.applied[2 * b] = di; a.applied[2 * b + 1] = ai;
+                a.state[4 * b] = x; a.state[4 * b + 1] = y; a.state[4 * b + 2] = v; a.state[4 * b + 3] = th;
+            }
+        }
+    } else if (pred_wave) {
+        di = a.applied[2 * b]; ai = a.applied[2 * b + 1];
+    }
+    if (pred_wave) {
+        if (!in) return;
+        double *row = a.obs6 + 6 * (size_t)b;
+        row[0] = x; row[1] = y; row[2] = v; row[3] = th; row[4] = ai; row[5] = di;
+        predict_row<false>(a.ip, x, y, v, th, ai, di, nullptr, a.pred + (size_t)b * a.ip.pred_steps * 4);
+        return;
+    }
+    if (in) rollout_group(a.p, x, y, v, th, failed ? nullptr : a.u + (size_t)b * 2 * T, j, s_roll + (size_t)r * RS);
+    __builtin_amdgcn_fence(__ATOMIC_RELEASE, "wavefront");
+    __builtin_amdgcn_wave_barrier();
+    __builtin_amdgcn_fence(__ATOMIC_ACQUIRE, "wavefront");
+    constexpr int ROWS = WAVE / G;
+    const int lane = tid & 63, r0 = (tid >> 6) * ROWS;
+    const int nr = n - r0 < ROWS ? n - r0 : ROWS;
+    double *out = a.xbar + (size_t)(b0 + r0) * 4 * W;
+    for (int i = lane; i < nr * 4 * W; i += WAVE) {
+        const int row = i / (4 * W);
+        out[i] = s_roll[(size_t)(r0 + row) * RS + (i - row * 4 * W)];
+    }
 }
 
 }
@@ -296,6 +376,13 @@
     if (retire && (!x.scatter || !x.queue_len))
         return mpcx_fail(ctx, MPCX_E_INVALID, "mpc_prepare_batch: retirement needs the queue order built beside the window selection");
     const bool forked = x.rollout_forked;
+    if (x.rollout_done) {
+        constexpr int per_block = mpcx::PREP_WAVES * mpcx::WIN_AGENTS;
+        const dim3 wgrid((B + per_block - 1) / per_block), wblock(64 * mpcx::PREP_WAVES);
+        if (retire) hipLaunchKernelGGL(mpcx::ref_window_kernel<true>, wgrid, wblock, 0, ctx->stream, ra);
+        else hipLaunchKernelGGL(mpcx::ref_window_kernel<false>, wgrid, wblock, 0, ctx->stream, ra);
+        return mpcx_check_launch(ctx, "prepare kernels");
+    }
     if (!forked) {
         int32_t rc = mpcx_rollout_fork(ctx, B, state, u_warm, xbar, x.done);
         if (rc != MPCX_OK) return rc;
@@ -326,6 +413,24 @@
     return MPCX_OK;
 }
 
+int32_t mpcx_head_enqueue(mpcx_ctx *ctx, const mpcx_interaction_params *ip, int32_t P, double *state, double *applied, double *u,
+                          const int32_t *status, const int32_t *iters, double *xbar, double *obs6, bool plant, bool reset_bins) {
+    if (!ctx || !ip || P <= 0 || !state || !applied || !u || !status || !iters || !xbar || !obs6 || !ctx->pred || !ctx->stats)
+        return mpcx_fail(ctx, MPCX_E_INVALID, "closed_loop_run: null pointer at the head of a step");
+    if (ctx->pred_cap < (size_t)P * ip->pred_steps * 4 * sizeof(double) || ctx->stats_slots < ((size_t)P + 63) / 64)
+        return mpcx_fail(ctx, MPCX_E_INVALID, "closed_loop_run: the prediction scratch or the statistics are too small for %d agents", P);
+    if (ctx->tune && ctx->tune_rows != P)
+        return mpcx_fail(ctx, MPCX_E_INVALID, "plant_step_batch: %d tuning rows are set but the batch has %d agents", ctx->tune_rows, P);
+    const bool rz = plant && reset_bins && ctx->bins && ctx->ticket;
+    mpcx::HeadArgs ha{ctx->mpc, *ip, P, state, applied, u, xbar, obs6, ctx->pred, status, iters, ctx->tune, ctx->stats,
+                      rz ? ctx->bins : nullptr, rz ? ctx->ticket : nullptr};
+    const size_t lds = mpcx::rollout_lds(ctx->mpc.T);
+    const dim3 grid((P + mpcx::ROLL_AGENTS - 1) / mpcx::ROLL_AGENTS), block(mpcx::HEAD_BLOCK);
+    if (plant) hipLaunchKernelGGL(mpcx::head_kernel<true>, grid, block, lds, ctx->stream, ha);
+    else hipLaunchKernelGGL(mpcx::head_kernel<false>, grid, block, lds, ctx->stream, ha);
+    return mpcx_check_launch(ctx, "head_kernel");
+}
+
 extern "C" int32_t mpcx_plant_step_batch(mpcx_ctx *ctx, int32_t B, double *state, double *u,
                                          const int32_t *status, double *applied) {
     return mpcx_plant_enqueue(ctx, B, state, u, status, applied, {});
diff --git a/mpc_for_av_at_intersection_amd/runtime.py b/mpc_for_av_at_intersection_amd/runtime.py
--- a/mpc_for_av_at_intersection_amd/runtime.py
+++ b/mpc_for_av_at_intersection_amd/runtime.py
@@ -738,6 +738,9 @@
         self._chk(self.lib.mpcx_set_linearisation_passes(self._ctx, int(passes)))
         self.lin_passes = int(passes)
 
+    def set_step_fusion(self, on: bool):
+        self._chk(self.lib.mpcx_set_step_fusion(self._ctx, 1 if on else 0))
+
     def profile_qp(self, enable: bool):
         self._chk(self.lib.mpcx_profile_qp(self._ctx, 1 if enable else 0))
 
```
